# uber-research/UPSNet

Hardware: NVIDIA H100
Metric: panoptic images/sec at 1024x2048 (higher is better)
Workload: dtype bf16x3

## Files before the change

include/upsnet_b200.h:

```cpp
#ifndef UPSNET_B200_H_
#define UPSNET_B200_H_

#include <stddef.h>
#include <stdint.h>

#ifdef __cplusplus
extern "C" {
#endif

#define UPSNET_E_BADARG (-1)
#define UPSNET_E_UNSUPPORTED (-2)
#define UPSNET_E_WORKSPACE (-3)

#define UPSNET_LAYOUT_NCHW 0
#define UPSNET_LAYOUT_NHWC 1
#define UPSNET_LAYOUT_FLAT_PAIR 2

#define UPSNET_DTYPE_F32 0
#define UPSNET_DTYPE_BF16 1
#define UPSNET_DTYPE_PAIR 2

#define UPSNET_EPI_RELU 1
#define UPSNET_EPI_RES_UP2 2
#define UPSNET_EPI_STEM_PAIR 8
#define UPSNET_EPI_NO_TMA 4
#define UPSNET_EPI_PAIR_GROUP(G) ((((G) / 64) & 0xfff) << 8)
#define UPSNET_EPI_SIGMOID_FROM(c) ((((c) + 1) & 0x3ff) << 20)

#define UPSNET_PREC_FP32_SIMT 0
#define UPSNET_PREC_BF16X3 1
#define UPSNET_PREC_BF16 2

int upsnet_version(int *n_sm);

int upsnet_roi_align_forward(const void *feat, int B, int C, int H, int W, int layout, int dtype,
                             const float *rois, int R, int PH, int PW, int sampling_ratio,
                             float spatial_scale, void *out, void *stream);

int upsnet_roi_align_fpn_forward(const void *const feats[4], const int Hs[4], const int Ws[4],
                                 const float scales[4], int B, int C, int layout, int dtype,
                                 const float *rois, int R, int PH, int PW, int sampling_ratio,
                                 void *out, int *levels_out, const int *n_dev, void *stream);

int upsnet_nms_workspace_bytes(int S, int max_seg_len, size_t *bytes);
int upsnet_nms_segmented(const float *boxes, const int *seg_offsets, int S, int max_seg_len,
                         float thresh, int *keep_out, int *keep_cnt, void *workspace,
                         size_t workspace_bytes, void *stream);
int upsnet_nms_host(int *keep_out, int *num_out, const float *boxes_host, int boxes_num,
                    int boxes_dim, float thresh, int device_id);

int upsnet_dcn_forward(const float *x, const float *offset, const float *mask,
                       const float *weight, const float *bias, float *y, int N, int Cin, int H,
                       int W, int Cout, int kh, int kw, int stride_h, int stride_w, int pad_h,
                       int pad_w, int dil_h, int dil_w, int deformable_groups, int epi_flags,
                       int precision, void *stream);

int upsnet_conv2d_forward(const float *x, const float *weight, const float *bias,
                          const float *residual, float *y, int N, int Cin, int H, int W,
                          int Cout, int kh, int kw, int stride_h, int stride_w, int pad_h,
                          int pad_w, int dil_h, int dil_w, int epi_flags, int precision,
                          void *stream);

int upsnet_igemm_packed_weight_bytes(int Cout, int Cin, int kh, int kw, size_t *bytes);
int upsnet_igemm_pack_weight(const float *weight, int Cout, int Cin, int kh, int kw, void *packed,
                             void *stream);
int upsnet_igemm_forward(const void *x_nhwc, const float *offset, const float *mask,
                         const void *packed, const float *bias, const void *residual, void *y,
                         int N, int H, int W, int Cin, int Cout, int kh, int kw, int stride_h,
                         int stride_w, int pad_h, int pad_w, int dil_h, int dil_w, int out_layout,
                         int x_dtype, int y_dtype, int epi_flags, int precision, const int *n_dev, void *stream);
int upsnet_tma_set_tile_n(int bn);

int upsnet_dcn_packed_weight_bytes(int Cout, int Cin, int kh, int kw, size_t *bytes);
int upsnet_dcn_pack_weight(const float *weight, int Cout, int Cin, int kh, int kw, void *packed, void *stream);
int upsnet_dcn_pair_forward(const void *x_pair, const float *offset, const float *mask, const void *packed,
                            const float *bias, void *y_pair, int N, int H, int W, int Cin, int Cout, int kh, int kw,
                            int pad_h, int pad_w, int dil_h, int dil_w, int epi_flags, void *stream);
int upsnet_dcn_set_tile_n(int bn);

int upsnet_panoptic_workspace_bytes(int n, int H, int W, int num_thing, size_t *bytes);
int upsnet_panoptic_workspace_min_bytes(int n, int H, int W, int num_thing, size_t *bytes);
int upsnet_panoptic_head(const float *fcn, int S, int H, int W, const float *boxes,
                         const float *cls_prob, const float *mask_logit, const int64_t *cls_idx,
                         int n, const int *n_dev, int num_stuff, double fraction_threshold, int64_t *keep_out,
                         int *k_out, int64_t *labels, int64_t *sem_labels, void *workspace,
                         size_t workspace_bytes, void *stream);
int upsnet_panoptic_head_up4(const float *score, int S, int Hs, int Ws, const float *boxes,
                             const float *cls_prob, const float *mask_logit, const int64_t *cls_idx,
                             int n, const int *n_dev, int num_stuff, double fraction_threshold, int64_t *keep_out,
                             int *k_out, int64_t *labels, int64_t *sem_labels, void *workspace,
                             size_t workspace_bytes, void *stream);

int upsnet_mask_removal(const float *boxes, const float *cls_prob, const float *mask_logit,
                        const int64_t *cls_idx, int n, const int *n_dev, int H, int W, int num_thing,
                        double fraction_threshold, int64_t *keep_out, int *k_out, float *mask_energy,
                        void *workspace, size_t workspace_bytes, void *stream);

int upsnet_stem_workspace_bytes(int N, int H, int W, int kh, int kw, int pad, size_t *bytes);
int upsnet_stem_packed_weight_bytes(int Cout, int kh, size_t *bytes);
int upsnet_stem_pack_weight(const float *weight, int Cout, int Cin, int kh, int kw, void *packed,
                            void *stream);
int upsnet_stem_forward(const float *x, const void *packed_w, const float *bias, void *y, int N, int Cin,
                        int H, int W, int Cout, int kh, int kw, int pad, int epi_flags, void *workspace,
                        size_t workspace_bytes, void *stream);

int upsnet_maxpool2d_nhwc(const void *x, void *y, int N, int H, int W, int C, int k, int stride,
                          int pad, int dtype, void *stream);

int upsnet_upsample_bilinear_nchw(const float *x, float *y, int planes, int H, int W, int factor,
                                  void *stream);

int upsnet_fcn_score_fuse(const float *s2, const float *s3, const float *s4, const float *s5, float *out,
                          int planes, int H, int W, void *stream);

int upsnet_fcn_score_fuse_backward(const float *dscore, float *ds3, float *ds4, float *ds5, int planes, int H,
                                   int W, void *stream);

int upsnet_rpn_decode(const float *const *deltas, const long long *const *top_idx, const int *k,
                      const int *hs, const int *ws, const int *strides, const double *base_anchors,
                      int L, int A, const float *im_info, float *boxes_out, void *stream);

int upsnet_rpn_topk_workspace_bytes(int L, size_t *bytes);
int upsnet_rpn_topk(const float *const *probs, const int *hs, const int *ws, int L, int A,
                    int pre_nms_top_n, float *out_scores, long long *out_idx, void *workspace,
                    size_t workspace_bytes, void *stream);

int upsnet_rpn_collect(const int *keep, const int *keep_cnt, const int *seg_offsets, const float *boxes,
                       const float *scores, int S, int max_seg_len, int post_nms_top_n, float *rois,
                       float *out_scores, unsigned char *valid, void *stream);

int upsnet_maskroi_prepare(const float *rois, const unsigned char *roi_valid, const float *bbox_delta,
                           const float *cls_prob, int R, int C, int class_agnostic, float score_thresh,
                           const float weights[4], const float *im_info, float *sc_out, int *cls_out,
                           float *bx_out, int *offs_out, void *stream);

int upsnet_maskroi_finish(const int *keep, const int *keep_cnt, const int *seg_offsets, const float *sc,
                          const int *cls, const float *bx, int nseg, int max_seg_len, int top_n, int cap,
                          float *out_sc, float *out_bx, long long *out_cls, int *n_out, void *stream);

int upsnet_mask_rows(const float *b1, const int *n1, int cap1, const float *b2, const int *n2, int cap2, float *rows,
                     int *u, int *pan_row, void *stream);

int upsnet_unified_pan_workspace_bytes(int num_seg_classes, size_t *bytes);
int upsnet_unified_pan_result(const long long *seg, const long long *pan, const long long *cls_inds, int k,
                              const int *k_dev, int H, int W, int num_seg_classes, int num_classes,
                              int stuff_area_limit, unsigned char *pan_2ch, int *err_out, void *workspace,
                              size_t workspace_bytes, void *stream);

int upsnet_prep_image(const unsigned char *image_hwc, int h, int w, double scale, int out_h, int out_w, int pad_h,
                      int pad_w, const double pixel_means[3], float *blob, int flip, void *stream);

int upsnet_label_restore(const long long *src0, const long long *src1, int Hp, int Wp, int h, int w, double fx,
                         int out_h, int out_w, long long *dst0, long long *dst1, void *stream);

#define UPSNET_PQ_MAX_GT 4096
#define UPSNET_PQ_MAX_PAIRS 65536
#define UPSNET_PQ_MAX_PRED 2048
#define UPSNET_PQ_E_PRED_CATEGORY 1
#define UPSNET_PQ_E_GT_COUNT 2
#define UPSNET_PQ_E_PAIRS 4
#define UPSNET_PQ_E_GT_TABLE 8
#define UPSNET_PQ_E_PRED_COUNT 16
#define UPSNET_PQ_E_MATCHES 32
int upsnet_pq_workspace_bytes(size_t *bytes);
int upsnet_pq_update(const unsigned char *pan_2ch, const unsigned char *gt_rgb, int H, int W, const long long *gt_table,
                     int num_gt, const unsigned char *cat_flags, long long *acc_counts, double *acc_iou, int *err,
                     void *workspace, size_t workspace_bytes, void *stream);

#define UPSNET_SSEG_MAX_CLASSES 224
int upsnet_sseg_update(const void *pred, int pred_bytes, int pred_pitch, const int *row_src, const int *col_src,
                       const unsigned char *gt, int H, int W, int num_classes, long long *acc, void *stream);

#define UPSNET_COCOEVAL_MAX_DET 2048
#define UPSNET_COCOEVAL_MAX_GT 1024
#define UPSNET_COCOEVAL_MAX_GT_CAT 192
#define UPSNET_COCOEVAL_MAX_CATEGORIES 256
#define UPSNET_COCOEVAL_MAX_IMAGES (1 << 17)
#define UPSNET_COCOEVAL_E_DET_COUNT 1
#define UPSNET_COCOEVAL_E_GT_COUNT 2
#define UPSNET_COCOEVAL_E_GT_CAT 4
#define UPSNET_COCOEVAL_E_CLASS 8
#define UPSNET_COCOEVAL_E_RECORDS 16
#define UPSNET_COCOEVAL_E_RLE_SIZE 32
typedef struct {
  float score;
  int category;
  int image;
  int rank;
  unsigned long long matched, ignored;
} upsnet_coco_record;
int upsnet_cocoeval_workspace_bytes(int n, int cap, long long gt_counts_total, size_t *bytes);
int upsnet_cocoeval_image(int segm, const float *boxes, const float *scores, const int64_t *cls_inds, int n,
                          const int *n_dev, const uint32_t *counts, int cap, const int *run_len, int H, int W,
                          const double *gt_table, int num_gt, const uint32_t *gt_counts, const int64_t *gt_offsets,
                          int num_categories, const int *class_to_k, int image_slot, upsnet_coco_record *records,
                          int record_cap, int *n_records, long long *npig, int *err, void *workspace,
                          size_t workspace_bytes, void *stream);
#define UPSNET_GT_RLE_E_CAPACITY 64
int upsnet_gt_rle_workspace_bytes(int num_anns, int h, int w, size_t *bytes);
int upsnet_gt_rle(int h, int w, int num_anns, const int *ann_poly, const int *poly_vert, const double *verts,
                  const int64_t *src_offsets, const uint32_t *src_counts, uint32_t *gt_counts, long long capacity,
                  int64_t *gt_offsets, int *err, void *workspace, size_t workspace_bytes, void *stream);
int upsnet_cocoeval_accumulate_workspace_bytes(int n_records, size_t *bytes);
int upsnet_cocoeval_accumulate(const upsnet_coco_record *records, int n_records, const int *image_rank,
                               const long long *npig, int num_categories, double *precision, double *recall,
                               double *scores, void *workspace, size_t workspace_bytes, void *stream);

#define UPSNET_COMBINED_MAX_DET 2048
#define UPSNET_COMBINED_E_RUN_LEN 1
#define UPSNET_COMBINED_E_RLE_SIZE 2
#define UPSNET_COMBINED_E_DET_COUNT 4
int upsnet_combined_pan_workspace_bytes(int n, int H, int W, size_t *bytes);
int upsnet_combined_pan_result(const void *sem, int sem_elem_size, int H, int W, const float *scores,
                               const int64_t *cls_inds, int n, const int *n_dev, const uint32_t *counts, int cap,
                               const int *run_len, int num_seg_classes, int num_classes, float score_threshold,
                               float fraction_threshold, int stuff_area_limit, unsigned char *pan_2ch, int *err,
                               void *workspace, size_t workspace_bytes, void *stream);

int upsnet_im_post_workspace_bytes(int n, int cap, size_t *bytes);
int upsnet_im_post_rle(const float *mask_probs, int C, int M, const float *boxes, const int64_t *cls_inds, int n,
                       const int *n_dev, int H, int W, uint32_t *counts, int cap, int *run_len, int *overflow,
                       void *workspace, size_t workspace_bytes, void *stream);

int upsnet_dcn_im2col(const float *x, const float *offset, const float *mask, int Cin, int H, int W, int kh, int kw,
                      int stride_h, int stride_w, int pad_h, int pad_w, int dil_h, int dil_w, float *col, void *stream);
int upsnet_dcn_col2im(const float *dcol, const float *offset, const float *mask, int Cin, int H, int W, int kh, int kw,
                      int stride_h, int stride_w, int pad_h, int pad_w, int dil_h, int dil_w, float *dx, void *stream);
int upsnet_dcn_col2im_coord(const float *dcol, const float *x, const float *offset, const float *mask, int Cin, int H,
                            int W, int kh, int kw, int stride_h, int stride_w, int pad_h, int pad_w, int dil_h, int dil_w,
                            float *doffset, float *dmask, void *stream);

int upsnet_roi_align_backward(const float *dout, const float *rois, int R, int B, int C, int H, int W, int PH, int PW,
                              int sampling_ratio, float spatial_scale, float *dfeat, void *stream);

#define UPSNET_RPN_TARGETS_MAX_G 4096
int upsnet_rpn_targets_workspace_bytes(long long num_anchors, int batch_size, size_t *bytes);
int upsnet_rpn_targets(const float *gt_boxes, int G, const double *cell_anchors, const int *strides,
                       const int *field_sizes, int L, int A, double im_height, double im_width, double straddle_thresh,
                       float positive_overlap, float negative_overlap, int batch_size, int num_fg, unsigned long long seed,
                       int64_t *labels, float *bbox_targets, float *inside_weights, float *outside_weights, int *counts,
                       void *workspace, size_t workspace_bytes, void *stream);

int upsnet_proposal_targets_workspace_bytes(int num_rois, int num_gt, int batch_rois, size_t *bytes);
int upsnet_proposal_targets(const float *rois, int R, const float *gt_boxes, const float *gt_max_overlaps,
                            const int *gt_max_classes, const int *gt_classes, const int *gt_box_to_gt_ind, int G,
                            const float *obj_boxes, const int *obj_poly_off, const int *poly_vert_off, const float *verts,
                            int num_objects, float im_scale, int num_classes, int batch_rois, int fg_per_image,
                            float fg_thresh, float bg_thresh_hi, float bg_thresh_lo, float wx, float wy, float ww,
                            float wh, int cls_agnostic_bbox_reg, int mask_size, unsigned long long seed, float *rois_out,
                            int64_t *labels, float *bbox_targets, float *bbox_inside_weights,
                            float *bbox_outside_weights, int64_t *nongt_inds, float *mask_rois, float *mask_int32,
                            unsigned char *roi_has_mask, int *counts, void *workspace, size_t workspace_bytes,
                            void *stream);

int upsnet_panoptic_loss_workspace_bytes(int k, int h, int w, size_t *bytes);
int upsnet_panoptic_loss_forward(const float *fcn_score, int S, int h, int w, const float *mask_score, int k, int C,
                                 int mask_size, const float *gt_rois, const int64_t *cls_idx, const int64_t *seg_gt,
                                 const void *mask_gt, int mask_gt_is_int64, int G, const int64_t *keep_inds,
                                 int num_classes, int enable_void, float box_scale, float *loss, float *accuracy,
                                 int *counts, float *lse, int *gt_channel, void *workspace, size_t workspace_bytes,
                                 void *stream);
int upsnet_panoptic_loss_backward(const float *fcn_score, int S, int h, int w, const float *mask_score, int k, int C,
                                  int mask_size, const float *gt_rois, const int64_t *cls_idx, int num_classes,
                                  int enable_void, float box_scale, const float *lse, const int *gt_channel,
                                  const float *grad_out, float *d_fcn_score, float *d_mask_score, void *workspace,
                                  size_t workspace_bytes, void *stream);

int upsnet_panoptic_gt(const int64_t *seg_gt, const void *mask_gt, int mask_gt_is_int64, int G, const int64_t *keep_inds,
                       int k, int h, int w, int num_seg_classes, int num_classes, int64_t *panoptic_gt, void *stream);

int upsnet_draw_keys(unsigned long long seed, int stream_id, int n, unsigned long long *keys, void *stream);

int upsnet_semantic_loss_workspace_bytes(int h, int w, size_t *bytes);
int upsnet_semantic_loss_forward(const float *fcn_score, int S, int h, int w, const void *seg_gt, int seg_gt_is_int64,
                                 float *loss, int *counts, float *lse, void *workspace, size_t workspace_bytes,
                                 void *stream);
int upsnet_semantic_loss_backward(const float *fcn_score, int S, int h, int w, const void *seg_gt, int seg_gt_is_int64,
                                  const float *lse, const int *counts, const float *grad_out, float *d_fcn_score,
                                  void *stream);

int upsnet_fcn_roi_loss_workspace_bytes(int S, int R, int M, int backward, size_t *bytes);
int upsnet_fcn_roi_loss_forward(const float *fcn_score, const float *bias, int S, int h, int w, const float *rois, int R,
                                const void *seg_roi_gt, int seg_roi_gt_is_int64, int M, int sampling_ratio,
                                float spatial_scale, float *loss, int *counts, float *lse, void *workspace,
                                size_t workspace_bytes, void *stream);
int upsnet_fcn_roi_loss_backward(const float *fcn_score, const float *bias, int S, int h, int w, const float *rois, int R,
                                 const void *seg_roi_gt, int seg_roi_gt_is_int64, int M, int sampling_ratio,
                                 float spatial_scale, const float *lse, const float *grad_out, float *d_fcn_score,
                                 float *d_bias, void *workspace, size_t workspace_bytes, void *stream);

int upsnet_rpn_loss_workspace_bytes(int num_anchors, size_t *bytes);
int upsnet_rpn_loss_forward(int num_levels, int A, const int *h, const int *w, const float *const *cls_score,
                            const float *const *bbox_pred, const int64_t *const *labels, const long long *label_strides,
                            const float *const *bbox_targets, const float *const *bbox_inside_weights,
                            const float *const *bbox_outside_weights, const long long *bbox_strides,
                            float rpn_batch_size, float *cls_loss, float *bbox_loss, void *workspace,
                            size_t workspace_bytes, void *stream);
int upsnet_rpn_loss_backward(int num_levels, int A, const int *h, const int *w, const float *const *cls_score,
                             const float *const *bbox_pred, const int64_t *const *labels, const long long *label_strides,
                             const float *const *bbox_targets, const float *const *bbox_inside_weights,
                             const float *const *bbox_outside_weights, const long long *bbox_strides,
                             float rpn_batch_size, const float *grad_cls, const float *grad_bbox,
                             float *const *d_cls_score, float *const *d_bbox_pred, void *stream);

int upsnet_mask_rcnn_loss_workspace_bytes(int R, int B, long long mask_numel, size_t *bytes);
int upsnet_mask_rcnn_loss_forward(const float *cls_score, const int64_t *cls_label, int R, int K, const float *bbox_pred,
                                  const float *bbox_target, const float *bbox_inside_weight,
                                  const float *bbox_outside_weight, int B, const float *mask_score,
                                  const float *mask_target, long long mask_numel, float *cls_loss, float *bbox_loss,
                                  float *mask_loss, float *accuracy, int *counts, void *workspace,
                                  size_t workspace_bytes, void *stream);
int upsnet_mask_rcnn_loss_backward(const float *cls_score, const int64_t *cls_label, int R, int K, const float *bbox_pred,
                                   const float *bbox_target, const float *bbox_inside_weight,
                                   const float *bbox_outside_weight, int B, const float *mask_score,
                                   const float *mask_target, long long mask_numel, const int *counts,
                                   const float *grad_cls, const float *grad_bbox, const float *grad_mask,
                                   float *d_cls_score, float *d_bbox_pred, float *d_mask_score, void *stream);

#define UPSNET_LABELS_MAX_POLY_VERTS 1024
#define UPSNET_LABELS_MAX_OBJ_VERTS 1536
#define UPSNET_LABELS_MAX_G 65535
int upsnet_training_labels(const unsigned char* label, int h0, int w0, const int* seg_rows, int Hs, const int* seg_cols,
                           int Ws, int64_t* seg_gt, const int* q_rows, int Hq, const int* q_cols, int Wq,
                           int64_t* seg_gt_4x, const int* m_rows, int Hm, const int* m_cols, int Wm, const int* obj_poly,
                           const int* poly_vert, const int* verts, const int* obj_yrange, int G, int max_poly_verts,
                           int max_obj_verts, void* mask_gt, int mask_gt_is_int64, const int* roi_rows,
                           const int* roi_cols, int n_roi, int M, int64_t* seg_roi_gt, void* stream);

#define UPSNET_SGD_MAX_GROUPS 16
#define UPSNET_SGD_CHUNK 8192
#define UPSNET_SGD_GRAD_F32 0
#define UPSNET_SGD_GRAD_BF16 1
#define UPSNET_SGD_GRAD_NONE 2
typedef struct {
  float *param;
  float *buf;
  const void *grad;
  int n;
  int group;
  int kind;
  float inv_world;
} upsnet_sgd_chunk;
typedef struct {
  const float *grad;
  void *out;
  int n;
  int reserved;
} upsnet_sgd_pack_chunk;
int upsnet_sgd_apply(const upsnet_sgd_chunk *chunks, int num_chunks, int num_groups, const double *group_lr,
                     const float *group_weight_decay, const float *group_momentum, double lr, const double *lr_table,
                     const unsigned char *decay_table, const int *iteration, int table_begin, int table_len,
                     void *stream);
int upsnet_sgd_pack(const upsnet_sgd_pack_chunk *chunks, int num_chunks, void *stream);
int upsnet_sgd_advance(int *iteration, void *stream);

#define UPSNET_GRAD_RELU 1
#define UPSNET_GRAD_RES_UP2 2
#define UPSNET_GRAD_UNSHUFFLE2 4
#define UPSNET_GRAD_DY_NHWC 8
int upsnet_conv_grad_prepare_workspace_bytes(int N, int C, int H, int W, int flags, size_t *bytes);
int upsnet_conv_grad_prepare(const float *dy, const float *y, void *g, float *dbias, float *dres, int N, int C, int H,
                             int W, int flags, int precision, void *workspace, size_t workspace_bytes, void *stream);
int upsnet_igemm_packed_weight_dgrad_bytes(int Cout, int Cin, int kh, int kw, size_t *bytes);
int upsnet_igemm_pack_weight_dgrad(const float *weight, int Cout, int Cin, int kh, int kw, void *packed, void *stream);
int upsnet_conv_dgrad_scatter2(const float *dxc, float *dx, int N, int H, int W, int C, void *stream);
int upsnet_conv_wgrad_workspace_bytes(int N, int H, int W, int Cin, int Cout, int kh, int kw, int stride_h, int stride_w,
                                      int pad_h, int pad_w, int dil_h, int dil_w, int precision, size_t *bytes);
int upsnet_conv_wgrad(const void *x_nhwc, const void *g, float *dw, int N, int H, int W, int Cin, int Cout, int kh, int kw,
                      int stride_h, int stride_w, int pad_h, int pad_w, int dil_h, int dil_w, int flags, int precision,
                      void *workspace, size_t workspace_bytes, void *stream);

int upsnet_group_norm_workspace_bytes(int N, int C, int H, int W, int groups, size_t *bytes);
int upsnet_group_norm_forward(const void *x, const float *gamma, const float *beta, const float *shift,
// ... 14 lines not shown
```

upsnet_b200/csrc/capi.cu:

```cuda
#include "common.cuh"
#include "tc_params.cuh"

namespace ups {
struct ConvParams {
  const float* x; const float* offset; const float* mask; const float* weight;
  const float* bias; const float* residual; float* y;
  int N, Cin, H, W, Cout, kh, kw, sh, sw, ph, pw, dh, dw, dg, Ho, Wo, relu;
};
int launch_igemm_simt(const ConvParams& p, cudaStream_t stream);

}

extern "C" int upsnet_version(int* n_sm) {
  if (n_sm) {
    int dev = 0, sms = 0;
    if (cudaGetDevice(&dev) == cudaSuccess &&
        cudaDeviceGetAttribute(&sms, cudaDevAttrMultiProcessorCount, dev) == cudaSuccess)
      *n_sm = sms;
    else
      *n_sm = -1;
  }
  return 90;
}

static int conv_common(const float* x, const float* offset, const float* mask, const float* weight,
                       const float* bias, const float* residual, float* y, int N, int Cin, int H,
                       int W, int Cout, int kh, int kw, int sh, int sw, int ph, int pw, int dh,
                       int dw, int dg, int epi_flags, int precision, void* stream) {
  if (!x || !weight || !y) return UPSNET_E_BADARG;
  if (N <= 0 || Cin <= 0 || H <= 0 || W <= 0 || Cout <= 0 || kh <= 0 || kw <= 0 || sh <= 0 ||
      sw <= 0 || ph < 0 || pw < 0 || dh <= 0 || dw <= 0 || dg <= 0 || Cin % dg != 0)
    return UPSNET_E_BADARG;
  ups::ConvParams p;
  p.x = x; p.offset = offset; p.mask = mask; p.weight = weight; p.bias = bias;
  p.residual = residual; p.y = y;
  p.N = N; p.Cin = Cin; p.H = H; p.W = W; p.Cout = Cout; p.kh = kh; p.kw = kw; p.sh = sh;
  p.sw = sw; p.ph = ph; p.pw = pw; p.dh = dh; p.dw = dw; p.dg = dg;
  p.Ho = ups::conv_out_size(H, ph, dh, kh, sh);
  p.Wo = ups::conv_out_size(W, pw, dw, kw, sw);
  p.relu = (epi_flags & UPSNET_EPI_RELU) ? 1 : 0;
  if (p.Ho <= 0 || p.Wo <= 0) return UPSNET_E_BADARG;
  if ((size_t)Cin * H * W >= (1ull << 31)) return UPSNET_E_UNSUPPORTED;
  switch (precision) {
    case UPSNET_PREC_FP32_SIMT:
      return ups::launch_igemm_simt(p, (cudaStream_t)stream);
    default:
      return UPSNET_E_UNSUPPORTED;
  }
}

extern "C" int upsnet_dcn_forward(const float* x, const float* offset, const float* mask,
                                  const float* weight, const float* bias, float* y, int N, int Cin,
                                  int H, int W, int Cout, int kh, int kw, int stride_h,
                                  int stride_w, int pad_h, int pad_w, int dil_h, int dil_w,
                                  int deformable_groups, int epi_flags, int precision,
                                  void* stream) {
  if (!offset) return UPSNET_E_BADARG;
  return conv_common(x, offset, mask, weight, bias, nullptr, y, N, Cin, H, W, Cout, kh, kw,
                     stride_h, stride_w, pad_h, pad_w, dil_h, dil_w, deformable_groups, epi_flags,
                     precision, stream);
}

extern "C" int upsnet_conv2d_forward(const float* x, const float* weight, const float* bias,
                                     const float* residual, float* y, int N, int Cin, int H, int W,
                                     int Cout, int kh, int kw, int stride_h, int stride_w,
                                     int pad_h, int pad_w, int dil_h, int dil_w, int epi_flags,
                                     int precision, void* stream) {
  return conv_common(x, nullptr, nullptr, weight, bias, residual, y, N, Cin, H, W, Cout, kh, kw,
                     stride_h, stride_w, pad_h, pad_w, dil_h, dil_w, 1, epi_flags, precision,
                     stream);
}

extern "C" int upsnet_igemm_packed_weight_bytes(int Cout, int Cin, int kh, int kw, size_t* bytes) {
  if (!bytes || Cout <= 0 || Cin <= 0 || kh <= 0 || kw <= 0) return UPSNET_E_BADARG;
  if (!ups::tc_supported(Cin, kh, kw, 1)) return UPSNET_E_UNSUPPORTED;
  *bytes = ups::tc_packed_weight_bytes(Cout, Cin, kh, kw);
  return 0;
}

extern "C" int upsnet_igemm_pack_weight(const float* weight, int Cout, int Cin, int kh, int kw,
                                        void* packed, void* stream) {
  if (!weight || !packed || Cout <= 0 || Cin <= 0 || kh <= 0 || kw <= 0) return UPSNET_E_BADARG;
  if (!ups::tc_supported(Cin, kh, kw, 1)) return UPSNET_E_UNSUPPORTED;
  return ups::tc_pack_weight(weight, Cout, Cin, kh, kw, packed, (cudaStream_t)stream);
}

extern "C" int upsnet_igemm_forward(const void* x_nhwc, const float* offset, const float* mask,
                                    const void* packed, const float* bias, const void* residual,
                                    void* y, int N, int H, int W, int Cin, int Cout, int kh, int kw,
                                    int stride_h, int stride_w, int pad_h, int pad_w, int dil_h,
                                    int dil_w, int out_layout, int x_dtype, int y_dtype, int epi_flags,
                                    int precision, const int* n_dev, void* stream) {
  if (!x_nhwc || !packed || !y) return UPSNET_E_BADARG;
  if (N <= 0 || Cin <= 0 || H <= 0 || W <= 0 || Cout <= 0 || kh <= 0 || kw <= 0 || stride_h <= 0 ||
      stride_w <= 0 || pad_h < 0 || pad_w < 0 || dil_h <= 0 || dil_w <= 0)
    return UPSNET_E_BADARG;
  if (precision != UPSNET_PREC_BF16X3 && precision != UPSNET_PREC_BF16) return UPSNET_E_BADARG;
  if (out_layout != UPSNET_LAYOUT_NCHW && out_layout != UPSNET_LAYOUT_NHWC) return UPSNET_E_BADARG;
  if (mask && !offset) return UPSNET_E_BADARG;
  if ((size_t)H * W >= (1ull << 31)) return UPSNET_E_UNSUPPORTED;
  ups::TcParams p{};
  p.x = x_nhwc; p.offset = offset; p.mask = mask; p.bias = bias; p.residual = residual; p.y = y;
  p.n_dev = n_dev;
  p.N = N; p.H = H; p.W = W; p.Cin = Cin; p.Cout = Cout; p.kh = kh; p.kw = kw; p.sh = stride_h;
  p.sw = stride_w; p.ph = pad_h; p.pw = pad_w; p.dh = dil_h; p.dw = dil_w;
  p.Ho = ups::conv_out_size(H, pad_h, dil_h, kh, stride_h);
  p.Wo = ups::conv_out_size(W, pad_w, dil_w, kw, stride_w);
  if (p.Ho <= 0 || p.Wo <= 0) return UPSNET_E_BADARG;
  p.relu = (epi_flags & UPSNET_EPI_RELU) ? 1 : 0;
  p.out_nhwc = out_layout == UPSNET_LAYOUT_NHWC;
  p.res_up2 = (epi_flags & UPSNET_EPI_RES_UP2) ? 1 : 0;
  p.no_tma = (epi_flags & UPSNET_EPI_NO_TMA) ? 1 : 0;
  if (p.res_up2 && (!residual || !p.out_nhwc || (p.Ho & 1) || (p.Wo & 1))) return UPSNET_E_BADARG;
  p.x3 = precision == UPSNET_PREC_BF16X3;
  if (x_dtype < UPSNET_DTYPE_F32 || x_dtype > UPSNET_DTYPE_PAIR || y_dtype < UPSNET_DTYPE_F32 || y_dtype > UPSNET_DTYPE_PAIR)
    return UPSNET_E_BADARG;
  p.x_bf16 = x_dtype == UPSNET_DTYPE_BF16;
  p.y_bf16 = y_dtype == UPSNET_DTYPE_BF16;
  p.x_pair = x_dtype == UPSNET_DTYPE_PAIR;
  p.y_pair = y_dtype == UPSNET_DTYPE_PAIR;
  p.pair_group = 64 * ((epi_flags >> 8) & 0xfff);
  p.sig_from = ((epi_flags >> 20) & 0x3ff) - 1;
  if (p.sig_from >= 0 && (p.y_pair || p.y_bf16 || p.residual)) return UPSNET_E_UNSUPPORTED;
  if (p.x_bf16 && p.x3) return UPSNET_E_UNSUPPORTED;
  if ((p.x_pair || p.y_pair) && !p.x3) return UPSNET_E_UNSUPPORTED;
  if (p.y_pair && !p.out_nhwc) return UPSNET_E_BADARG;
  return ups::launch_igemm_tc(p, packed, (cudaStream_t)stream);
}
```

upsnet_b200/csrc/igemm_tma.cu:

```cuda
#include <cuda.h>
#include <cuda_bf16.h>
#include <cstdlib>

#include "common.cuh"
#include "tc_ptx.cuh"
#include "tc_params.cuh"

namespace ups {

constexpr int TM_EPI_WARPS = 8;
constexpr int TM_WARP_TMA = 8, TM_WARP_RES = 9;
constexpr int TM_THREADS = 10 * 32;
constexpr int TM_MAX_STAGES = 8;
constexpr int TM_SLAB_BYTES = 128 * 128;
constexpr int TM_MMA_BF16 = 0, TM_MMA_WIDE = 1;

struct TmaGeom {
  const float* bias;
  int N, Ho, Wo, Cout, Cin;
  int kw, KHW, ph, pw, dh, dw;
  int bw, bh, bn;
  int tiles_w, tiles_h, tiles_n, n_tiles;
  const int* n_dev;
  int BN, stages, relu, has_res;
  int res_up2;
  int direct, y_bf16, out_nhwc;
  void* y;
  int stem;
  int sig_from;
  int x3;
  int x_lo;
  int w_lo;
  int pg;
  int res_inplace;
  int opairs;
  int wide;
};

__device__ __forceinline__ int pair_chan(int n, int G) { return (n / G) * 2 * G + (n % G); }

struct TmaSmem {
  uint32_t stages, out, res, acc, a_bytes, b_bytes, stage_bytes, total;
  uint32_t a_half, b_half;
  uint32_t oslabs, res_slab;
};
template <int N, int W>
__device__ __forceinline__ void acc_stage_sw(const float (&d)[N / 2], float* buf, int row0) {
  const int t = threadIdx.x & 127, l = t & 31;
  const int r = row0 + 16 * (t >> 5) + (l >> 2);
#pragma unroll
  for (int i = 0; i < W / 8; ++i) {
    const int c = 8 * i + 2 * (l & 3);
#pragma unroll
    for (int h = 0; h < 2; ++h) {
      const int rr = r + 8 * h;
      const int pc = ((((c >> 2) ^ (rr & 7))) << 2) | (c & 3);
      *reinterpret_cast<float2*>(buf + (size_t)rr * W + pc) = make_float2(d[4 * i + 2 * h], d[4 * i + 2 * h + 1]);
    }
  }
}
__device__ __forceinline__ void acc_ld16_sw(uint32_t rowaddr, int row, int col, uint32_t (&r)[16]) {
#pragma unroll
  for (int i = 0; i < 4; ++i) {
    const uint32_t a = rowaddr + ((uint32_t)(((col >> 2) + i) ^ (row & 7)) << 4);
    asm volatile("ld.shared.v4.b32 {%0, %1, %2, %3}, [%4];"
                 : "=r"(r[4 * i]), "=r"(r[4 * i + 1]), "=r"(r[4 * i + 2]), "=r"(r[4 * i + 3]) : "r"(a));
  }
}
__host__ __device__ inline TmaSmem tma_smem_layout(int BN, int stages, bool has_res, bool direct, bool x3, bool res_up2,
                                                  bool res_inplace, int opairs) {
  TmaSmem s;
  const uint32_t mul = x3 ? 2u : 1u;
  s.a_half = 128 * 128; s.b_half = (uint32_t)BN * 128;
  s.a_bytes = s.a_half * mul;
  s.b_bytes = s.b_half * mul;
  s.stage_bytes = s.a_bytes + s.b_bytes;
  s.stages = 1024;
  s.out = s.stages + s.stage_bytes * (uint32_t)stages;
  s.res_slab = (x3 && res_up2) ? 4096u : (uint32_t)TM_SLAB_BYTES;
  if (x3) {
    s.oslabs = direct ? 0u : (res_inplace ? 2u * (uint32_t)(BN / 64) : (uint32_t)opairs);
    s.res = s.out + s.oslabs * 2u * TM_SLAB_BYTES;
    s.acc = s.res + ((has_res && !res_inplace) ? 2u * (uint32_t)(BN / 64) * 2u * s.res_slab : 0u);
  } else {
    s.oslabs = 0;
    const uint32_t out_slabs = direct ? 0 : (BN == 64 ? 1 : 2);
    s.res = s.out + out_slabs * TM_SLAB_BYTES;
    s.acc = s.res + (has_res ? 2u * (uint32_t)(BN / 64) * TM_SLAB_BYTES : 0u);
  }
  s.total = s.acc + ((x3 && !direct) ? 0u : 128u * (uint32_t)BN * 4u);
  return s;
}

template <int N, int MMA>
__global__ void __launch_bounds__(TM_THREADS, 1)
igemm_tma_kernel(const __grid_constant__ CUtensorMap tm_x, const __grid_constant__ CUtensorMap tm_w,
                 const __grid_constant__ CUtensorMap tm_y, const __grid_constant__ CUtensorMap tm_r, const TmaGeom g) {
  extern __shared__ __align__(1024) uint8_t smem_dyn[];
  const uint32_t raw = smem_u32(smem_dyn);
  const uint32_t base = (raw + 1023u) & ~1023u;
  uint8_t* sm = smem_dyn + (base - raw);
  const TmaSmem L = tma_smem_layout(g.BN, g.stages, g.has_res != 0, g.direct != 0, g.x3 != 0, g.res_up2 != 0, g.res_inplace != 0,
                                    g.opairs);
  const uint32_t bar_full = base, bar_empty = base + 8 * TM_MAX_STAGES;
  const uint32_t bar_rfull = bar_empty + 8 * TM_MAX_STAGES, bar_rempty = bar_rfull + 16;

  const int tid = threadIdx.x, warp = tid >> 5, lane = tid & 31;
  const int cchunks = g.Cin / 64;
  const int num_kb = g.KHW * cchunks;
  const int tiles_n = g.n_dev ? (min(max(*g.n_dev, 0), g.N) + g.bn - 1) / g.bn : g.tiles_n;
  const long long m_tiles = (long long)g.tiles_w * g.tiles_h * tiles_n;
  const long long num_tiles = m_tiles * g.n_tiles;
  const uint32_t box_bytes = (uint32_t)(g.bw * g.bh * g.bn) * 128u;

  if (tid == 0) {
    for (int s = 0; s < g.stages; ++s) {
      mbar_init(bar_full + 8 * s, 1);
      mbar_init(bar_empty + 8 * s, TM_EPI_WARPS);
    }
    for (int b = 0; b < 2; ++b) {
      mbar_init(bar_rfull + 8 * b, 1);
      mbar_init(bar_rempty + 8 * b, g.res_inplace ? 1 : TM_EPI_WARPS);
    }
    fence_mbar_init();
  } else if (warp == TM_WARP_TMA && lane == 0) {
    prefetch_tmap(&tm_x);
    prefetch_tmap(&tm_w);
    prefetch_tmap(&tm_y);
    if (g.has_res || (g.stem && g.x3)) prefetch_tmap(&tm_r);
  }
  __syncthreads();

  if (warp == TM_WARP_TMA) {
    if (lane == 0) {
      uint32_t s = 0, ph = 0;
      uint32_t a_dst = base + L.stages;
      const uint32_t tx_bytes = (g.x3 ? 2u * box_bytes : box_bytes) + L.b_bytes;
      for (long long tile = blockIdx.x; tile < num_tiles; tile += gridDim.x) {
        const int nt = (int)(tile % g.n_tiles);
        const long long mt = tile / g.n_tiles;
        const int w0 = (int)(mt % g.tiles_w) * g.bw;
        const int h0 = (int)((mt / g.tiles_w) % g.tiles_h) * g.bh;
        const int i0 = (int)(mt / ((long long)g.tiles_w * g.tiles_h)) * g.bn;
        const int n0 = nt * g.BN;
        int kbr = 0, cc = 0, kj = 0;
        int cw = w0 - g.pw, ch = h0 - g.ph;
        for (int kb = 0; kb < num_kb; ++kb) {
          const uint32_t bf = bar_full + 8 * s;
          mbar_wait(bar_empty + 8 * s, ph ^ 1u);
          mbar_arrive_expect_tx(bf, tx_bytes);
          if (g.stem)
            tma_load_5d(a_dst, &tm_x, bf, 0, w0, kbr & 1, h0 + (kbr >> 1), i0);
          else
            tma_load_4d(a_dst, &tm_x, bf, cc * 64, cw, ch, i0);
          tma_load_2d(a_dst + L.a_bytes, &tm_w, bf, kbr * 64, n0);
          if (g.x3) {
            if (g.stem)
              tma_load_5d(a_dst + L.a_half, &tm_r, bf, 0, w0, kbr & 1, h0 + (kbr >> 1), i0);
            else
              tma_load_4d(a_dst + L.a_half, &tm_x, bf, g.x_lo + cc * 64, cw, ch, i0);
            tma_load_2d(a_dst + L.a_bytes + L.b_half, &tm_w, bf, kbr * 64, g.w_lo + n0);
          }
          ++kbr;
          if (++cc == cchunks) {
            cc = 0; cw += g.dw;
            if (++kj == g.kw) { kj = 0; cw = w0 - g.pw; ch += g.dh; }
          }
          a_dst += L.stage_bytes;
          if (++s == (uint32_t)g.stages) { s = 0; ph ^= 1u; a_dst = base + L.stages; }
        }
      }
    }
    __syncwarp();
  } else if (warp == TM_WARP_RES) {
    if (lane == 0 && g.has_res) {
      uint32_t ti_local = 0;
      const int slabs = g.BN / 64;
      for (long long tile = blockIdx.x; tile < num_tiles; tile += gridDim.x, ++ti_local) {
        const int nt = (int)(tile % g.n_tiles);
        const long long mt = tile / g.n_tiles;
        const int w0 = (int)(mt % g.tiles_w) * g.bw;
        const int h0 = (int)((mt / g.tiles_w) % g.tiles_h) * g.bh;
        const int i0 = (int)(mt / ((long long)g.tiles_w * g.tiles_h)) * g.bn;
        const uint32_t rb = ti_local & 1u, ruse = ti_local >> 1;
        const uint32_t rdst = base + L.res + rb * (uint32_t)slabs * TM_SLAB_BYTES;
        mbar_wait(bar_rempty + 8 * rb, (ruse & 1u) ^ 1u);
        if (g.x3) {
          const uint32_t lo_off = g.res_inplace ? (uint32_t)TM_SLAB_BYTES : L.res_slab;
          const uint32_t pdst = g.res_inplace ? base + L.out + rb * (uint32_t)slabs * 2u * TM_SLAB_BYTES
                                              : base + L.res + rb * (uint32_t)slabs * 2u * L.res_slab;
          mbar_arrive_expect_tx(bar_rfull + 8 * rb, (g.res_up2 ? box_bytes / 4 : box_bytes) * (uint32_t)slabs * 2u);
          for (int s = 0; s < slabs; ++s) {
            const int c = pair_chan(nt * g.BN + s * 64, g.pg);
            tma_load_4d(pdst + (uint32_t)s * 2u * lo_off, &tm_r, bar_rfull + 8 * rb, c, w0 >> g.res_up2, h0 >> g.res_up2, i0);
            tma_load_4d(pdst + (uint32_t)s * 2u * lo_off + lo_off, &tm_r, bar_rfull + 8 * rb, c + g.pg, w0 >> g.res_up2,
                        h0 >> g.res_up2, i0);
          }
          continue;
        }
        mbar_arrive_expect_tx(bar_rfull + 8 * rb, (g.res_up2 ? box_bytes / 4 : box_bytes) * (uint32_t)slabs);
        for (int s = 0; s < slabs; ++s)
          tma_load_4d(rdst + s * TM_SLAB_BYTES, &tm_r, bar_rfull + 8 * rb, nt * g.BN + s * 64, w0 >> g.res_up2,
                      h0 >> g.res_up2, i0);
      }
    }
    __syncwarp();
  } else {
    const int wg = warp >> 2;
    const uint32_t dhi = wg_desc_hi(1024);
    const uint32_t a_row0 = (uint32_t)wg * 64u * 128u;
    const uint32_t ah16 = L.a_half >> 4;
    float* accbuf = reinterpret_cast<float*>(sm + L.acc);
    constexpr int SW = MMA == TM_MMA_WIDE ? N / 2 : N;
    const bool staged = MMA != TM_MMA_WIDE || g.direct;
    float d[N / 2];
    uint32_t s = 0, ph = 0;
    auto mainloop = [&]() {
      int prev = -1;
      for (int kb = 0; kb < num_kb; ++kb) {
        mbar_wait(bar_full + 8 * s, ph);
        const uint32_t st0 = base + L.stages + s * L.stage_bytes;
        const uint32_t a = wg_desc_lo(st0 + a_row0), b = wg_desc_lo(st0 + L.a_bytes);
        wgmma_fence();
#pragma unroll
        for (uint32_t k = 0; k < 4; ++k) {
          const uint32_t acc = (kb | k) ? 1u : 0u;
          if constexpr (MMA == TM_MMA_WIDE) {
            Wgmma<N>::mma(d, wg_desc(a + 2 * k, dhi), wg_desc(b + 2 * k, dhi), acc);
            Wgmma<N / 2>::mma(*reinterpret_cast<float(*)[N / 4]>(&d[0]), wg_desc(a + ah16 + 2 * k, dhi), wg_desc(b + 2 * k, dhi), 1u);
          } else {
            Wgmma<N>::mma(d, wg_desc(a + 2 * k, dhi), wg_desc(b + 2 * k, dhi), acc);
          }
        }
        wgmma_commit();
        wgmma_wait<1>();
        wgmma_fence_acc(d);
        if (prev >= 0 && lane == 0) mbar_arrive(bar_empty + 8 * prev);
        prev = (int)s;
        if (++s == (uint32_t)g.stages) { s = 0; ph ^= 1u; }
      }
      wgmma_wait<0>();
      wgmma_fence_acc(d);
      if (prev >= 0 && lane == 0) mbar_arrive(bar_empty + 8 * prev);
      if constexpr (MMA == TM_MMA_WIDE) {
#pragma unroll
        for (int i = 0; i < N / 4; ++i) { d[i] += d[N / 4 + i]; d[N / 4 + i] = 0.f; }
      }
      if (staged) {
        named_bar(3, 256);
        acc_stage_sw<N, SW>(d, accbuf, wg * 64);
        named_bar(3, 256);
      }
    };
    const int q = warp & 3, half = warp >> 2;
    const int row = q * 32 + lane;
    const uint32_t trow = smem_u32(accbuf + (size_t)row * SW);
    const int units = g.BN / 32;
    const int upw = units >= 4 ? units / 2 : 1;
    const int bar_id = g.BN == 64 ? 1 : 1 + half;
    const int bar_cnt = g.BN == 64 ? 256 : 128;
    const bool leader = (g.BN == 64 ? warp == 0 : q == 0) && lane == 0;
    const uint32_t out_slab = base + L.out + (g.BN == 64 ? 0u : (uint32_t)half * TM_SLAB_BYTES);
    const uint32_t sw_row = (uint32_t)row * 128u;
    const uint32_t rx = (uint32_t)(row & 7);
    auto res_row = [&](int r) {
      if (!g.res_up2) return r;
      const int w = r % g.bw, h = (r / g.bw) % g.bh, n = r / (g.bw * g.bh);
      return (w >> 1) + (g.bw >> 1) * ((h >> 1) + (g.bh >> 1) * n);
    };
    const int rrow = res_row(row);
    const uint32_t rs_row = (uint32_t)rrow * 128u, rrx = (uint32_t)(rrow & 7);
    uint32_t fr_row[2], fr_res[2], fr_rx[2];
#pragma unroll
    for (int h = 0; h < 2; ++h) {
      const int r = wg * 64 + 16 * (warp & 3) + (lane >> 2) + 8 * h, rr = res_row(r);
      fr_row[h] = (uint32_t)r * 128u; fr_res[h] = (uint32_t)rr * 128u; fr_rx[h] = (uint32_t)(rr & 7);
    }
    uint32_t ti_local = 0, oc = 0;
    for (long long tile = blockIdx.x; tile < num_tiles; tile += gridDim.x, ++ti_local) {
      const int nt = (int)(tile % g.n_tiles);
      const long long mt = tile / g.n_tiles;
      const int w0 = (int)(mt % g.tiles_w) * g.bw;
      const int h0 = (int)((mt / g.tiles_w) % g.tiles_h) * g.bh;
      const int i0 = (int)(mt / ((long long)g.tiles_w * g.tiles_h)) * g.bn;
      const int n0 = nt * g.BN;
      const uint32_t buf = ti_local & 1u, use = ti_local >> 1;
      mainloop();
      if (g.has_res) mbar_wait(bar_rfull + 8 * buf, use & 1u);
      if (g.direct) {
        const int wq = row % g.bw, hq = (row / g.bw) % g.bh, nq = row / (g.bw * g.bh);
        const int wo = w0 + wq, ho = h0 + hq, ni = i0 + nq;
        const bool ok = nq < g.bn && wo < g.Wo && ho < g.Ho && ni < g.N;
        const size_t HoWo = (size_t)g.Ho * g.Wo;
        const size_t pix = ((size_t)ni * g.Ho + ho) * g.Wo + wo;
        const int cbeg = half * (g.BN / 2), cend = cbeg + g.BN / 2;
        for (int cb = cbeg; cb < cend; cb += 16) {
          uint32_t v[16];
          acc_ld16_sw(trow, row, cb, v);
          const int co0 = n0 + cb;
          if (!ok || co0 >= g.Cout) continue;
#pragma unroll
          for (int e = 0; e < 16; ++e) {
            const int co = co0 + e;
            if (co >= g.Cout) break;
            float o = __uint_as_float(v[e]);
            if (g.bias) o += __ldg(g.bias + co);
            if (g.relu) o = fmaxf(o, 0.f);
            if (g.sig_from >= 0 && co >= g.sig_from) o = 1.f / (1.f + expf(-o));
            const size_t oi = g.out_nhwc ? pix * g.Cout + co : ((size_t)ni * g.Cout + co) * HoWo + (size_t)ho * g.Wo + wo;
            if (g.y_bf16) reinterpret_cast<__nv_bfloat16*>(g.y)[oi] = __float2bfloat16_rn(o);
            else reinterpret_cast<float*>(g.y)[oi] = o;
          }
        }
        continue;
      }
      if constexpr (MMA == TM_MMA_WIDE) {
        const bool lead = warp == 0 && lane == 0;
        const uint32_t cq4 = (uint32_t)(lane & 3) * 4u;
        const uint32_t fx = (uint32_t)(lane >> 2);
#pragma unroll
        for (int sl = 0; sl < SW / 64; ++sl, ++oc) {
          uint32_t ob;
          if (g.res_inplace) {
            ob = base + L.out + (buf * (uint32_t)(SW / 64) + (uint32_t)sl) * 2u * TM_SLAB_BYTES;
          } else {
            ob = base + L.out + (g.opairs == 2 ? (oc & 1u) : 0u) * 2u * TM_SLAB_BYTES;
            if (lead) {
              if (g.opairs == 2) bulk_wait_read1(); else bulk_wait_read0();
            }
            named_bar(1, 256);
          }
#pragma unroll
          for (int j = 0; j < 8; ++j) {
            const int i = 8 * sl + j;
            float2 bv = make_float2(0.f, 0.f);
            if (g.bias) bv = __ldg(reinterpret_cast<const float2*>(g.bias + n0 + 8 * i) + (lane & 3));
#pragma unroll
            for (int h = 0; h < 2; ++h) {
              float a = d[4 * i + 2 * h], b = d[4 * i + 2 * h + 1];
              const uint32_t oa = ob + fr_row[h] + (((uint32_t)j ^ fx) << 4) + cq4;
              if (g.bias) { a += bv.x; b += bv.y; }
              if (g.has_res) {
                uint32_t hw, lw;
                if (g.res_inplace) { hw = lds32(oa); lw = lds32(oa + TM_SLAB_BYTES); }
                else {
                  const uint32_t ra = base + L.res + (buf * (uint32_t)(SW / 64) + (uint32_t)sl) * 2u * L.res_slab + fr_res[h];
                  hw = lds32(ra + (((uint32_t)j ^ fr_rx[h]) << 4) + cq4);
                  lw = lds32(ra + L.res_slab + (((uint32_t)j ^ fr_rx[h]) << 4) + cq4);
                }
                a += pair_x(hw, lw);
                b += pair_y(hw, lw);
              }
              if (g.relu) { a = fmaxf(a, 0.f); b = fmaxf(b, 0.f); }
              uint32_t hw, lw;
              split_pair2(a, b, hw, lw);
              sts32(oa, hw);
              sts32(oa + TM_SLAB_BYTES, lw);
            }
          }
          fence_proxy_async();
          named_bar(1, 256);
          if (lead) {
            const int c = pair_chan(n0 + sl * 64, g.pg);
            tma_store_4d(&tm_y, ob, c, w0, h0, i0);
            tma_store_4d(&tm_y, ob + TM_SLAB_BYTES, c + g.pg, w0, h0, i0);
            bulk_commit();
          }
        }
        __syncwarp();
        if (lane == 0 && g.has_res && !g.res_inplace) mbar_arrive(bar_rempty + 8 * buf);
        if (g.res_inplace && lead) {
          bulk_wait_read0();
          mbar_arrive(bar_rempty + 8 * buf);
        }
      } else {
        for (int ui = 0; ui < upw; ++ui) {
          const int u = half * upw + ui;
          const int slab = u >> 1;
          const uint32_t jb = (uint32_t)(u & 1) * 4u;
          uint32_t v0[16], v1[16];
          acc_ld16_sw(trow, row, u * 32, v0);
          acc_ld16_sw(trow, row, u * 32 + 16, v1);
          if ((u & 1) == 0 || g.BN == 64) {
            if (leader) bulk_wait_read0();
            named_bar(bar_id, bar_cnt);
          }
          float o[32];
  #pragma unroll
          for (int e = 0; e < 16; ++e) { o[e] = __uint_as_float(v0[e]); o[16 + e] = __uint_as_float(v1[e]); }
          if (g.bias) {
            const float4* bp = reinterpret_cast<const float4*>(g.bias + n0 + u * 32);
  #pragma unroll
            for (int e = 0; e < 8; ++e) {
              const float4 b4 = __ldg(bp + e);
              o[4 * e] += b4.x; o[4 * e + 1] += b4.y; o[4 * e + 2] += b4.z; o[4 * e + 3] += b4.w;
            }
          }
          if (g.has_res) {
            const uint32_t rs = base + L.res + (buf * (uint32_t)(g.BN / 64) + (uint32_t)slab) * TM_SLAB_BYTES + rs_row;
  #pragma unroll
            for (int c = 0; c < 4; ++c) {
              const uint4 rv = lds128(rs + (((jb + c) ^ rrx) << 4));
              const uint32_t rw[4] = {rv.x, rv.y, rv.z, rv.w};
  #pragma unroll
              for (int e = 0; e < 4; ++e) {
                o[c * 8 + 2 * e] += bf16x2_x(rw[e]);
                o[c * 8 + 2 * e + 1] += bf16x2_y(rw[e]);
              }
            }
          }
          if (g.relu) {
  #pragma unroll
            for (int e = 0; e < 32; ++e) o[e] = fmaxf(o[e], 0.f);
          }
  #pragma unroll
          for (int c = 0; c < 4; ++c) sts128(out_slab + sw_row + (((jb + c) ^ rx) << 4), pack_bf16x8(o + c * 8));
          if ((u & 1) == 1 || g.BN == 64) {
            fence_proxy_async();
            named_bar(bar_id, bar_cnt);
            if (leader) {
              tma_store_4d(&tm_y, out_slab, n0 + slab * 64, w0, h0, i0);
              bulk_commit();
            }
          }
        }
        __syncwarp();
        if (lane == 0 && g.has_res) mbar_arrive(bar_rempty + 8 * buf);
      }
    }
    if (leader || (g.x3 && warp == 0 && lane == 0)) bulk_wait0();
  }
}

static bool encode_bf16(EncodeTiledFn enc, CUtensorMap* tm, const void* ptr, int rank, const cuuint64_t* dims,
                        const cuuint32_t* box, const cuuint64_t* byte_strides = nullptr) {
  cuuint64_t strides[5];
  cuuint64_t acc = 2;
  for (int i = 0; i + 1 < rank; ++i) { acc *= dims[i]; strides[i] = byte_strides ? byte_strides[i] : acc; }
  const cuuint32_t es[5] = {1, 1, 1, 1, 1};
  return enc(tm, CU_TENSOR_MAP_DATA_TYPE_BFLOAT16, (cuuint32_t)rank, const_cast<void*>(ptr), dims, strides, box, es,
             CU_TENSOR_MAP_INTERLEAVE_NONE, CU_TENSOR_MAP_SWIZZLE_128B, CU_TENSOR_MAP_L2_PROMOTION_L2_256B,
             CU_TENSOR_MAP_FLOAT_OOB_FILL_NONE) == CUDA_SUCCESS;
}

static void tma_pick_box(int N, int Ho, int Wo, int kh, int kw, int dh, int dw, bool even, int* bw_o, int* bh_o, int* bn_o) {
  long long best_tiles = -1, best_halo = 0;
  int bbw = 1, bbh = 1, bbn = 1;
  const int wmax = Wo < 128 ? Wo : 128;
  for (int bw = 1; bw <= wmax; ++bw) {
    if (Wo > 32 && (bw & (bw - 1))) continue;
    if (even && (bw & 1)) continue;
    const int hmax = (128 / bw) < Ho ? (128 / bw) : Ho;
    for (int bh = 1; bh <= hmax; ++bh) {
      if (even && (bh & 1)) continue;
      int bn = 128 / (bw * bh);
      if (bn > N) bn = N;
      if (bn < 1) continue;
      const long long tiles = (long long)((Wo + bw - 1) / bw) * ((Ho + bh - 1) / bh) * ((N + bn - 1) / bn);
      const long long halo = (long long)(bw + (kw - 1) * dw) * (bh + (kh - 1) * dh) * bn;
      if (best_tiles < 0 || tiles < best_tiles || (tiles == best_tiles && (halo < best_halo || (halo == best_halo && bw > bbw)))) {
        best_tiles = tiles; best_halo = halo; bbw = bw; bbh = bh; bbn = bn;
      }
    }
  }
  *bw_o = bbw; *bh_o = bbh; *bn_o = bbn;
}

template <int N, int MMA>
static int tma_launch_n(dim3 grid, size_t smem, cudaStream_t stream, const CUtensorMap& tm_x, const CUtensorMap& tm_w,
                        const CUtensorMap& tm_y, const CUtensorMap& tm_r, const TmaGeom& g) {
  static ups::PerDeviceOnce configured;
  if (configured.need())
    UPS_CUDA(cudaFuncSetAttribute(igemm_tma_kernel<N, MMA>, cudaFuncAttributeMaxDynamicSharedMemorySize, 227 * 1024));
  igemm_tma_kernel<N, MMA><<<grid, TM_THREADS, smem, stream>>>(tm_x, tm_w, tm_y, tm_r, g);
  UPS_CHECK_LAUNCH();
  return 0;
}
static int tma_launch(int BN, dim3 grid, size_t smem, cudaStream_t stream, const CUtensorMap& tm_x, const CUtensorMap& tm_w,
                      const CUtensorMap& tm_y, const CUtensorMap& tm_r, const TmaGeom& g) {
  if (g.wide) {
    if (BN == 32) return tma_launch_n<64, TM_MMA_WIDE>(grid, smem, stream, tm_x, tm_w, tm_y, tm_r, g);
    if (BN == 64) return tma_launch_n<128, TM_MMA_WIDE>(grid, smem, stream, tm_x, tm_w, tm_y, tm_r, g);
    if (BN == 128) return tma_launch_n<256, TM_MMA_WIDE>(grid, smem, stream, tm_x, tm_w, tm_y, tm_r, g);
  } else {
    if (BN == 32) return tma_launch_n<32, TM_MMA_BF16>(grid, smem, stream, tm_x, tm_w, tm_y, tm_r, g);
    if (BN == 64) return tma_launch_n<64, TM_MMA_BF16>(grid, smem, stream, tm_x, tm_w, tm_y, tm_r, g);
    if (BN == 128) return tma_launch_n<128, TM_MMA_BF16>(grid, smem, stream, tm_x, tm_w, tm_y, tm_r, g);
  }
  return UPSNET_E_UNSUPPORTED;
}

static bool tma_fit(int BN, bool has_res, bool direct, bool pair, bool res_up2, bool res_inplace, int* stages, int* opairs,
                    TmaSmem* L) {
  const uint32_t cap = 227 * 1024 - 1024;
  auto lay = [&](int st, int op) { return tma_smem_layout(BN, st, has_res, direct, pair, res_up2, res_inplace, op); };
  int st = TM_MAX_STAGES, op = 2;
  while (st > 2 && lay(st, op).total > cap) --st;
  if (pair && !direct && !res_inplace && (st < 4 || lay(st, op).total > cap)) {
    int st1 = 4;
    while (st1 > 2 && lay(st1, 1).total > cap) --st1;
    if (st1 > st || lay(st, op).total > cap) { st = st1; op = 1; }
  }
  *stages = st; *opairs = op; *L = lay(st, op);
  return L->total <= cap;
}

static int g_tma_force_bn = 0;

int launch_igemm_tma(const TcParams& p, const void* packed, cudaStream_t stream) {
  if (p.no_tma || p.offset) return UPSNET_E_UNSUPPORTED;
  const bool pair = p.x_pair != 0;
  if (pair != (p.x3 != 0) || (!pair && !p.x_bf16)) return UPSNET_E_UNSUPPORTED;
  if (p.y_pair && (!pair || !p.out_nhwc || (p.Cout % 64) != 0)) return UPSNET_E_UNSUPPORTED;
  if (pair && p.y_bf16) return UPSNET_E_UNSUPPORTED;
  const int pg = p.y_pair ? (p.pair_group > 0 ? p.pair_group : p.Cout) : 0;
  if (p.y_pair && ((pg % 64) != 0 || (p.Cout % pg) != 0)) return UPSNET_E_UNSUPPORTED;
  const bool direct = (!p.y_bf16 && !p.y_pair) || !p.out_nhwc || (p.Cout % 64) != 0;
  if (p.sig_from >= 0 && !direct) return UPSNET_E_UNSUPPORTED;
  if (direct && (p.residual || p.Cout > 256)) return UPSNET_E_UNSUPPORTED;
  if (p.res_up2 && (!p.residual || (p.Ho & 1) || (p.Wo & 1))) return UPSNET_E_UNSUPPORTED;
  const bool strided = p.sh != 1 || p.sw != 1;
  if (strided && (p.kh != 1 || p.kw != 1 || p.ph != 0 || p.pw != 0)) return UPSNET_E_UNSUPPORTED;
  if ((p.Cin % 64) || (!direct && (p.Cout % 64)) || p.kh * p.kw > 49) return UPSNET_E_UNSUPPORTED;
  if ((((uintptr_t)p.x) & 15) || (((uintptr_t)p.y) & 15) || (((uintptr_t)packed) & 15) || (p.residual && (((uintptr_t)p.residual) & 15)))
    return UPSNET_E_UNSUPPORTED;
  if (p.bias && (((uintptr_t)p.bias) & 15)) return UPSNET_E_UNSUPPORTED;
  EncodeTiledFn enc = tma_encoder();
  if (!enc) return UPSNET_E_UNSUPPORTED;
  const int sms = num_sms();
  TmaGeom g{};
  g.bias = p.bias;
  g.N = p.N; g.Ho = p.Ho; g.Wo = p.Wo; g.Cout = p.Cout; g.Cin = p.Cin;
  g.kw = p.kw; g.KHW = p.kh * p.kw; g.ph = p.ph; g.pw = p.pw; g.dh = p.dh; g.dw = p.dw;
  g.relu = p.relu; g.has_res = p.residual ? 1 : 0; g.res_up2 = p.res_up2 ? 1 : 0; g.sig_from = p.sig_from;
  g.n_dev = p.n_dev;
  tma_pick_box(p.N, p.Ho, p.Wo, p.kh, p.kw, p.dh, p.dw, g.res_up2 != 0, &g.bw, &g.bh, &g.bn);
  g.tiles_w = (p.Wo + g.bw - 1) / g.bw;
  g.tiles_h = (p.Ho + g.bh - 1) / g.bh;
  g.tiles_n = (p.N + g.bn - 1) / g.bn;
  const long long m_tiles = (long long)g.tiles_w * g.tiles_h * g.tiles_n;
  const int Cout_pad = cout_pad(p.Cout);
  int BN = (Cout_pad % 128 == 0) ? 128 : (Cout_pad % 64 == 0 ? 64 : 32);
  g.x3 = pair ? 1 : 0; g.x_lo = p.Cin; g.w_lo = Cout_pad; g.pg = pg;
  g.res_inplace = (pair && g.has_res && !g.res_up2) ? 1 : 0;
  g.opairs = 2;
  if (g_tma_force_bn && Cout_pad % g_tma_force_bn == 0) {
    BN = g_tma_force_bn;
  } else {
    while (BN > 64 && m_tiles * (Cout_pad / BN) < 88) BN /= 2;
  }
  g.direct = direct ? 1 : 0; g.y_bf16 = p.y_bf16; g.out_nhwc = p.out_nhwc; g.y = p.y;
  TmaSmem L;
  bool ok = tma_fit(BN, g.has_res != 0, direct, pair, g.res_up2 != 0, g.res_inplace != 0, &g.stages, &g.opairs, &L);
  while (BN > 64 && (!ok || (pair && g.stages < 3))) {
    BN /= 2;
    ok = tma_fit(BN, g.has_res != 0, direct, pair, g.res_up2 != 0, g.res_inplace != 0, &g.stages, &g.opairs, &L);
  }
  if (!ok) return UPSNET_E_UNSUPPORTED;
  g.BN = BN;
  g.n_tiles = Cout_pad / BN;

  const int Kp = g.KHW * p.Cin;
  CUtensorMap tm_x, tm_w, tm_y, tm_r;
  {
    const cuuint64_t xm = pair ? 2 : 1;
    const cuuint64_t dx[4] = {(cuuint64_t)p.Cin * xm, (cuuint64_t)(strided ? p.Wo : p.W), (cuuint64_t)(strided ? p.Ho : p.H),
                              (cuuint64_t)p.N};
    const cuuint64_t sx[3] = {(cuuint64_t)p.sw * p.Cin * 2 * xm, (cuuint64_t)p.sh * p.W * p.Cin * 2 * xm,
                              (cuuint64_t)p.H * p.W * p.Cin * 2 * xm};
    const cuuint64_t dy[4] = {(cuuint64_t)p.Cout * xm, (cuuint64_t)p.Wo, (cuuint64_t)p.Ho, (cuuint64_t)p.N};
    const cuuint64_t dwt[2] = {(cuuint64_t)Kp, (cuuint64_t)Cout_pad * xm};
    const cuuint32_t box[4] = {64, (cuuint32_t)g.bw, (cuuint32_t)g.bh, (cuuint32_t)g.bn};
    const cuuint32_t boxw[2] = {64, (cuuint32_t)BN};
    if (!encode_bf16(enc, &tm_x, p.x, 4, dx, box, sx)) return UPSNET_E_UNSUPPORTED;
    if (!encode_bf16(enc, &tm_w, packed, 2, dwt, boxw)) return UPSNET_E_UNSUPPORTED;
    if (direct) {
      tm_y = tm_x;
      tm_r = tm_x;
    } else {
    if (!encode_bf16(enc, &tm_y, p.y, 4, dy, box)) return UPSNET_E_UNSUPPORTED;
    if (g.res_up2) {
      const cuuint64_t dr[4] = {(cuuint64_t)p.Cout * xm, (cuuint64_t)(p.Wo / 2), (cuuint64_t)(p.Ho / 2), (cuuint64_t)p.N};
      const cuuint32_t boxr[4] = {64, (cuuint32_t)(g.bw / 2), (cuuint32_t)(g.bh / 2), (cuuint32_t)g.bn};
      if (!encode_bf16(enc, &tm_r, p.residual, 4, dr, boxr)) return UPSNET_E_UNSUPPORTED;
    } else if (!encode_bf16(enc, &tm_r, p.residual ? p.residual : p.y, 4, dy, box)) {
      return UPSNET_E_UNSUPPORTED;
    }
    }
  }
  const long long num_tiles = m_tiles * g.n_tiles;
  if (num_tiles <= 0) return 0;
  g.wide = pair ? 1 : 0;
  dim3 grid((unsigned)(num_tiles < sms ? num_tiles : sms));
  return tma_launch(BN, grid, L.total + 1024, stream, tm_x, tm_w, tm_y, tm_r, g);
}


__global__ void stem_pack_image_kernel(const float* __restrict__ x, uint4* __restrict__ xp, uint4* __restrict__ xp_lo, int N, int C,
                                       int H, int W, int pad, int Hp, int Wp) {
  const long long total = (long long)N * Hp * Wp;
  for (long long t = (long long)blockIdx.x * blockDim.x + threadIdx.x; t < total; t += (long long)gridDim.x * blockDim.x) {
    const int c = (int)(t % Wp);
    const long long rest = t / Wp;
    const int r = (int)(rest % Hp), n = (int)(rest / Hp);
    const int hi = r - pad, wi = c - pad;
    float v[8] = {0.f, 0.f, 0.f, 0.f, 0.f, 0.f, 0.f, 0.f};
    if (hi >= 0 && hi < H && wi >= 0 && wi < W)
      for (int ch = 0; ch < C; ++ch) v[ch] = __ldg(x + (((size_t)n * C + ch) * H + hi) * W + wi);
    const uint4 o = pack_bf16x8(v);
    xp[t] = o;
    if (xp_lo) xp_lo[t] = pair_lo8(v, o);
  }
}

__global__ void stem_pack_weight_kernel(const float* __restrict__ w, int Cout, int Cin, int kh, int kw,
                                        __nv_bfloat16* __restrict__ packed) {
  const int total = Cout * kh * 64;
  for (int i = blockIdx.x * blockDim.x + threadIdx.x; i < total; i += gridDim.x * blockDim.x) {
    const int c = i & 7, kx = (i >> 3) & 7, ky = (i >> 6) % kh, co = i / (64 * kh);
    const float v = (c < Cin && kx < kw) ? w[(((size_t)co * Cin + c) * kh + ky) * kw + kx] : 0.f;
    __nv_bfloat16 h, l;
    split_bf16(v, h, l);
    packed[i] = h;
    packed[total + i] = l;
  }
}

static void stem_geometry(int H, int W, int kh, int kw, int pad, int* Ho, int* Wo, int* Hp, int* Wp) {
  *Ho = (H + 2 * pad - kh) / 2 + 1;
  *Wo = (W + 2 * pad - kw) / 2 + 1;
  *Hp = 2 * (*Ho + (kh >> 1));
  *Wp = 2 * *Wo + 8;
}

inline size_t stem_layout(int N, int Hp, int Wp, bool pair, void* base, uint4** hi, uint4** lo) {
  WsCarve c(base);
  const size_t pixels = (size_t)N * Hp * Wp;
  *hi = c.take<uint4>(pixels);
  *lo = pair ? c.take<uint4>(pixels) : nullptr;
  return c.bytes();
}

}

extern "C" int upsnet_tma_set_tile_n(int bn) {
  if (bn != 0 && bn != 64 && bn != 128) return UPSNET_E_BADARG;
  ups::g_tma_force_bn = bn;
  return 0;
}

extern "C" int upsnet_stem_workspace_bytes(int N, int H, int W, int kh, int kw, int pad, size_t* bytes) {
  if (!bytes || N <= 0 || H <= 0 || W <= 0 || kh <= 0 || kw <= 0 || kw > 8 || pad < 0) return UPSNET_E_BADARG;
  int Ho, Wo, Hp, Wp;
  ups::stem_geometry(H, W, kh, kw, pad, &Ho, &Wo, &Hp, &Wp);
  if (Ho <= 0 || Wo <= 0) return UPSNET_E_BADARG;
  uint4 *hi, *lo;
  *bytes = ups::stem_layout(N, Hp, Wp, true, nullptr, &hi, &lo);
  return 0;
}

extern "C" int upsnet_stem_packed_weight_bytes(int Cout, int kh, size_t* bytes) {
  if (!bytes || Cout <= 0 || kh <= 0) return UPSNET_E_BADARG;
  *bytes = (size_t)Cout * kh * 64 * 2 * 2;
  return 0;
}

extern "C" int upsnet_stem_pack_weight(const float* weight, int Cout, int Cin, int kh, int kw, void* packed, void* stream) {
  if (!weight || !packed || Cout <= 0 || Cin <= 0 || Cin > 8 || kh <= 0 || kw <= 0 || kw > 8) return UPSNET_E_BADARG;
  const int total = Cout * kh * 64;
  ups::stem_pack_weight_kernel<<<(total + 255) / 256, 256, 0, (cudaStream_t)stream>>>(weight, Cout, Cin, kh, kw,
                                                                                         (__nv_bfloat16*)packed);
  UPS_CHECK_LAUNCH();
  return 0;
}

extern "C" int upsnet_stem_forward(const float* x, const void* packed_w, const float* bias, void* y, int N, int Cin, int H,
                                   int W, int Cout, int kh, int kw, int pad, int epi_flags, void* workspace,
                                   size_t workspace_bytes, void* stream) {
  using namespace ups;
  if (!x || !packed_w || !y || !workspace) return UPSNET_E_BADARG;
  if (N <= 0 || Cin <= 0 || Cin > 8 || H <= 0 || W <= 0 || kh <= 0 || kw <= 0 || kw > 8 || pad < 0) return UPSNET_E_BADARG;
  if ((Cout % 64) || Cout > 256 || kh > 16) return UPSNET_E_UNSUPPORTED;
  if ((((uintptr_t)y) & 15) || (((uintptr_t)packed_w) & 15) || (((uintptr_t)workspace) & 15)) return UPSNET_E_BADARG;
  if (bias && (((uintptr_t)bias) & 15)) return UPSNET_E_UNSUPPORTED;
  int Ho, Wo, Hp, Wp;
  stem_geometry(H, W, kh, kw, pad, &Ho, &Wo, &Hp, &Wp);
  if (Ho <= 0 || Wo <= 0) return UPSNET_E_BADARG;
  const bool pair = (epi_flags & UPSNET_EPI_STEM_PAIR) != 0;
  uint4 *x_hi, *x_lo;
  if (workspace_bytes < stem_layout(N, Hp, Wp, pair, workspace, &x_hi, &x_lo)) return UPSNET_E_WORKSPACE;
  EncodeTiledFn enc = tma_encoder();
  if (!enc) return UPSNET_E_UNSUPPORTED;
  cudaStream_t st = (cudaStream_t)stream;
  TmaGeom g{};
  g.bias = bias;
  g.N = N; g.Ho = Ho; g.Wo = Wo; g.Cout = Cout; g.Cin = 64;
  g.kw = 1; g.KHW = kh; g.ph = 0; g.pw = 0; g.dh = 1; g.dw = 1;
  g.relu = (epi_flags & UPSNET_EPI_RELU) ? 1 : 0;
  g.sig_from = -1;
  g.stem = 1; g.y = y; g.y_bf16 = 1; g.out_nhwc = 1;
  g.x3 = pair ? 1 : 0; g.w_lo = Cout; g.pg = Cout; g.opairs = 2; g.x_lo = 0;
  tma_pick_box(N, Ho, Wo, 1, 1, 1, 1, false, &g.bw, &g.bh, &g.bn);
  g.tiles_w = (Wo + g.bw - 1) / g.bw;
  g.tiles_h = (Ho + g.bh - 1) / g.bh;
  g.tiles_n = (N + g.bn - 1) / g.bn;
  g.BN = (Cout % 128 == 0 && !pair) ? 128 : 64;
  g.n_tiles = Cout / g.BN;
  g.wide = pair ? 1 : 0;
  TmaSmem L;
  if (!tma_fit(g.BN, false, false, pair, false, false, &g.stages, &g.opairs, &L)) return UPSNET_E_UNSUPPORTED;
  CUtensorMap tm_x, tm_w, tm_y, tm_lo;
  {
    const cuuint64_t pitch = (cuuint64_t)Wp * 16;
    const cuuint64_t dx[5] = {64, (cuuint64_t)Wo, 2, (cuuint64_t)(Hp / 2), (cuuint64_t)N};
    const cuuint64_t sx[4] = {32, pitch, 2 * pitch, (cuuint64_t)Hp * pitch};
    const cuuint32_t bx[5] = {64, (cuuint32_t)g.bw, 1, (cuuint32_t)g.bh, (cuuint32_t)g.bn};
    const cuuint64_t dwt[2] = {(cuuint64_t)kh * 64, (cuuint64_t)Cout * 2};
    const cuuint32_t bw2[2] = {64, (cuuint32_t)g.BN};
    const cuuint64_t dy[4] = {(cuuint64_t)Cout * (pair ? 2 : 1), (cuuint64_t)Wo, (cuuint64_t)Ho, (cuuint64_t)N};
    const cuuint32_t by[4] = {64, (cuuint32_t)g.bw, (cuuint32_t)g.bh, (cuuint32_t)g.bn};
    if (!encode_bf16(enc, &tm_x, x_hi, 5, dx, bx, sx)) return UPSNET_E_UNSUPPORTED;
    tm_lo = tm_x;
    if (pair && !encode_bf16(enc, &tm_lo, x_lo, 5, dx, bx, sx)) return UPSNET_E_UNSUPPORTED;
    if (!encode_bf16(enc, &tm_w, packed_w, 2, dwt, bw2)) return UPSNET_E_UNSUPPORTED;
    if (!encode_bf16(enc, &tm_y, y, 4, dy, by)) return UPSNET_E_UNSUPPORTED;
  }
  {
    const long long total = (long long)N * Hp * Wp;
    long long blocks = (total + 255) / 256;
    if (blocks > kNumSMs * 32) blocks = kNumSMs * 32;
    stem_pack_image_kernel<<<(unsigned)blocks, 256, 0, st>>>(x, x_hi, x_lo, N, Cin, H, W, pad, Hp, Wp);
    UPS_CHECK_LAUNCH();
  }
  const int sms = num_sms();
  const long long num_tiles = (long long)g.tiles_w * g.tiles_h * g.tiles_n * g.n_tiles;
  dim3 grid((unsigned)(num_tiles < sms ? num_tiles : sms));
  return tma_launch(g.BN, grid, L.total + 1024, st, tm_x, tm_w, tm_y, pair ? tm_lo : tm_y, g);
}
```

upsnet_b200/csrc/tc_params.cuh:

```cuda
#pragma once
#include <cuda.h>
#include <cuda_runtime.h>
#include <cstdint>

namespace ups {

inline int cout_pad(int Cout) { return Cout <= 32 ? 32 : (Cout + 63) / 64 * 64; }

typedef CUresult (*EncodeTiledFn)(CUtensorMap*, CUtensorMapDataType, cuuint32_t, void*, const cuuint64_t*, const cuuint64_t*,
                                  const cuuint32_t*, const cuuint32_t*, CUtensorMapInterleave, CUtensorMapSwizzle,
                                  CUtensorMapL2promotion, CUtensorMapFloatOOBfill);

inline EncodeTiledFn tma_encoder() {
  static EncodeTiledFn fn = nullptr;
  static bool tried = false;
  if (!tried) {
    void* p = nullptr;
    cudaDriverEntryPointQueryResult qr = cudaDriverEntryPointSymbolNotFound;
    if (cudaGetDriverEntryPoint("cuTensorMapEncodeTiled", &p, cudaEnableDefault, &qr) == cudaSuccess &&
        qr == cudaDriverEntryPointSuccess)
      fn = reinterpret_cast<EncodeTiledFn>(p);
    else
      (void)cudaGetLastError();
    tried = true;
  }
  return fn;
}

struct TcParams {
  const void* x;
  const float* offset;
  const float* mask;
  const uint16_t* w_hi;
  const uint16_t* w_lo;
  const float* bias; const void* residual; void* y;
  int N, H, W, Cin, Cout, Cout_pad, kh, kw, sh, sw, ph, pw, dh, dw, Ho, Wo;
  int relu, out_nhwc, BN, stages, x3;
  int x_bf16, y_bf16;
  int x_pair, y_pair;
  int sig_from;
  int pair_group;
  int res_up2;
  int no_tma;
  int tile_w, tile_h;
  const int* n_dev;
};

size_t tc_packed_weight_bytes(int Cout, int Cin, int kh, int kw);
int tc_pack_weight(const float* w, int Cout, int Cin, int kh, int kw, void* packed, cudaStream_t stream);
bool tc_supported(int Cin, int kh, int kw, int dg);
int launch_igemm_tc(TcParams p, const void* packed, cudaStream_t stream);
int launch_igemm_tma(const TcParams& p, const void* packed, cudaStream_t stream);

}
```

upsnet_b200/model.py:

```python
import math

import numpy as np
import torch
import torch.nn as nn
import torch.nn.functional as F

from . import _lib, training
from . import operators as ops
from .detection import MaskROI, ProposalGenerator, StaticMaskROI, StaticProposalGenerator
from .operators import DeformConv, DeformConvWithOffset


class UPSNetConfig:

    def __init__(self, **kw):
        self.num_classes = 9
        self.num_seg_classes = 19
        self.backbone_with_dconv = 100
        self.backbone_with_dilation = False
        self.backbone_with_dpyramid = False
        self.backbone_freeze_at = 2
        self.backbone_fix_bn = True
        self.fpn_feature_dim = 256
        self.fpn_with_gap = False
# ... 24 lines not shown
        self.fpn_with_norm = "none"
        self.rpn_with_norm = "none"
        self.rcnn_with_norm = "none"
        self.fcn_with_norm = "none"
        for k, v in kw.items():
            if not hasattr(self, k):
                raise AttributeError(k)
            setattr(self, k, v)

    @classmethod
    def from_reference_config(cls, config):
        def get(sec, key, default):
            d = config.get(sec, {}) if hasattr(config, "get") else getattr(config, sec, {})
            try:
                return d[key]
            except (KeyError, TypeError):
                return getattr(d, key, default)
        return cls(num_classes=int(get("dataset", "num_classes", 9)), num_seg_classes=int(get("dataset", "num_seg_classes", 19)),
                   backbone_with_dconv=int(get("network", "backbone_with_dconv", 100)),
                   backbone_with_dilation=bool(get("network", "backbone_with_dilation", False)),
                   backbone_with_dpyramid=bool(get("network", "backbone_with_dpyramid", False)),
                   backbone_freeze_at=int(get("network", "backbone_freeze_at", 2)),
                   backbone_fix_bn=bool(get("network", "backbone_fix_bn", True)),
                   fpn_feature_dim=int(get("network", "fpn_feature_dim", 256)), fpn_with_gap=bool(get("network", "fpn_with_gap", False)),
                   fcn_num_layers=int(get("network", "fcn_num_layers", 3)), num_anchors=int(get("network", "num_anchors", 3)),
                   anchor_scales=tuple(get("network", "anchor_scales", (8,))), anchor_ratios=tuple(get("network", "anchor_ratios", (0.5, 1, 2))),
                   rpn_feat_stride=tuple(get("network", "rpn_feat_stride", (4, 8, 16, 32, 64))), mask_size=int(get("network", "mask_size", 28)),
                   bbox_reg_weights=tuple(get("network", "bbox_reg_weights", (10., 10., 5., 5.))),
                   rpn_pre_nms_top_n=int(get("test", "rpn_pre_nms_top_n", 1000)), rpn_post_nms_top_n=int(get("test", "rpn_post_nms_top_n", 1000)),
                   rpn_nms_thresh=float(get("test", "rpn_nms_thresh", 0.7)), rpn_min_size=int(get("test", "rpn_min_size", 0)),
                   nms_thresh=float(get("test", "nms_thresh", 0.5)), max_det=int(get("test", "max_det", 100)),
                   score_thresh=float(get("test", "score_thresh", 0.05)), panoptic_score_thresh=float(get("test", "panoptic_score_thresh", 0.6)),
                   panoptic_box_keep_fraction=float(get("train", "panoptic_box_keep_fraction", 0.7)),
                   train_rpn_pre_nms_top_n=int(get("train", "rpn_pre_nms_top_n", 2000)),
                   train_rpn_post_nms_top_n=int(get("train", "rpn_post_nms_top_n", 2000)),
                   train_rpn_nms_thresh=float(get("train", "rpn_nms_thresh", 0.7)),
                   train_rpn_min_size=int(get("train", "rpn_min_size", 0)),
                   batch_rois=int(get("train", "batch_rois", 512)), rpn_batch_size=int(get("train", "rpn_batch_size", 256)),
                   fg_fraction=float(get("train", "fg_fraction", 0.25)),
                   fcn_with_roi_loss=bool(get("train", "fcn_with_roi_loss", False)),
                   **{k: str(get("network", k, "none")) for k in NORM_KEYS})

    @classmethod
    def cityscapes_r50(cls):
        return cls()

    @classmethod
    def coco_r50(cls):
        return cls(num_classes=81, num_seg_classes=133, fpn_with_gap=True, fcn_num_layers=3, fcn_with_roi_loss=True)

    @classmethod
    def coco_r101_dcn(cls):
        return cls(num_classes=81, num_seg_classes=133, backbone_with_dconv=3, fpn_with_gap=True,
                   fcn_num_layers=3, fcn_with_roi_loss=True)


NORM_KEYS = ("fpn_with_norm", "rpn_with_norm", "rcnn_with_norm", "fcn_with_norm")


def _check_norms(cfg):
    for k in NORM_KEYS:
        v = getattr(cfg, k)
        if v not in ("none", "group_norm", "batch_norm"):
            raise _lib.UpsnetError("network.%s: %r is not one of 'none', 'group_norm', 'batch_norm'" % (k, v))
        if v == "batch_norm" and k != "rpn_with_norm":
            raise _lib.UpsnetError("network.%s = 'batch_norm' is not built: the reference's BatchNorm2d comes from its "
                                   "absent distbatchnorm module (SyncBN); use 'group_norm' or 'none'" % k)


def _gn_conv(cin, cout, k, padding=0):
    return nn.Sequential(nn.Conv2d(cin, cout, k, padding=padding, bias=False), nn.GroupNorm(32, cout))


def _fold_bn(conv_w, bn):
    with torch.no_grad():
        scale = bn.weight / torch.sqrt(bn.running_var + bn.eps)
        shift = (bn.bias - bn.running_mean * scale).contiguous()
    return (conv_w * scale.view(-1, 1, 1, 1)).contiguous(), shift


class Bottleneck(nn.Module):

    def __init__(self, inplanes, planes, stride=1, dilation=1, downsample=None, deformable=False):
        super().__init__()
        self.conv1 = nn.Conv2d(inplanes, planes, 1, stride=stride, bias=False)
        self.bn1 = nn.BatchNorm2d(planes)
        self.deformable = deformable
        if deformable:
            self.conv2_offset = nn.Conv2d(planes, 18, 3, 1, 1)
            self.conv2_offset.weight.data.zero_()
            self.conv2_offset.bias.data.zero_()
            self.conv2 = DeformConv(planes, planes, 3, stride=1, padding=dilation, dilation=dilation, bias=False)
        else:
            self.conv2 = nn.Conv2d(planes, planes, 3, 1, dilation, dilation, bias=False)
        self.bn2 = nn.BatchNorm2d(planes)
        self.conv3 = nn.Conv2d(planes, planes * 4, 1, bias=False)
        self.bn3 = nn.BatchNorm2d(planes * 4)
        self.downsample = downsample
        self.stride, self.dilation = stride, dilation
        self._f = None

    def prepare(self):
        f = {}
        f["w1"], f["b1"] = _fold_bn(self.conv1.weight, self.bn1)
        f["w2"], f["b2"] = _fold_bn(self.conv2.weight, self.bn2)
        f["w3"], f["b3"] = _fold_bn(self.conv3.weight, self.bn3)
        if self.downsample is not None:
            f["wd"], f["bd"] = _fold_bn(self.downsample[0].weight, self.downsample[1])
        self._f = {k: v.detach() for k, v in f.items()}

    def forward(self, x):
        f = self._f
        out = ops.conv2d(x, f["w1"], f["b1"], stride=self.stride, relu=True)
        if self.deformable:
            offset = ops.conv2d(out, self.conv2_offset.weight, self.conv2_offset.bias, 1, 1, 1, out_format="nchw")
            out = ops.deform_conv(out, offset, f["w2"], f["b2"], 1, self.dilation, self.dilation, relu=True)
        else:
            out = ops.conv2d(out, f["w2"], f["b2"], 1, self.dilation, self.dilation, relu=True)
        residual = x if self.downsample is None else ops.conv2d(x, f["wd"], f["bd"], stride=self.stride)
        return ops.conv2d(out, f["w3"], f["b3"], residual=residual, relu=True)

    def forward_train(self, x, prec):
        w1, b1 = _fold_bn(self.conv1.weight, self.bn1)
        out = training.conv2d(x, w1, b1, stride=self.stride, relu=True, precision=prec)
        w2, b2 = _fold_bn(self.conv2.weight, self.bn2)
        if self.deformable:
            offset = training.OffsetConvFunction.apply(out, self.conv2_offset.weight, self.conv2_offset.bias)
            out = F.relu(training.DeformConvFunction.apply(out, offset, w2, b2, 1, self.dilation, self.dilation))
        else:
            out = training.conv2d(out, w2, b2, 1, self.dilation, self.dilation, relu=True, precision=prec)
        residual = x
        if self.downsample is not None:
            wd, bd = _fold_bn(self.downsample[0].weight, self.downsample[1])
            residual = training.conv2d(x, wd, bd, stride=self.stride, precision=prec)
        w3, b3 = _fold_bn(self.conv3.weight, self.bn3)
        return training.conv2d(out, w3, b3, residual=residual, relu=True, precision=prec)


class Stem(nn.Module):

    def __init__(self):
        super().__init__()
        self.conv1 = nn.Conv2d(3, 64, 7, 2, 3, bias=False)
        self.bn1 = nn.BatchNorm2d(64)
        self._f = None

    def prepare(self):
        w, b = _fold_bn(self.conv1.weight, self.bn1)
        self._f = (w.detach(), b.detach())

    def forward(self, x):
        stream = ops._stream()
        if x.is_cuda and stream != "f32":
            x = ops.stem_conv(x, self._f[0], self._f[1], 3, relu=True, pair=stream == "pair")
        else:
            x = ops.conv2d(x, self._f[0], self._f[1], stride=2, padding=3, relu=True)
        return ops.max_pool2d(x, 3, 2, 1)


class ResBlock(nn.Module):

    def __init__(self, planes, blocks, stride=1, dilation=1, deformable=False, with_dpyramid=False):
        super().__init__()
        inplanes = planes * 2 if planes != 64 else planes
        downsample = None
        if stride != 1 or inplanes != planes * 4:
            downsample = nn.Sequential(nn.Conv2d(inplanes, planes * 4, 1, stride=stride, bias=False),
                                       nn.BatchNorm2d(planes * 4))
        layers = [Bottleneck(inplanes, planes, stride, dilation, downsample, deformable)]
        for _ in range(1, blocks - 1):
            layers.append(Bottleneck(planes * 4, planes, dilation=dilation, deformable=deformable))
        layers.append(Bottleneck(planes * 4, planes, dilation=dilation, deformable=deformable or with_dpyramid))
        self.layers = nn.Sequential(*layers)

    def forward(self, x):
        return self.layers(x)


class ResNetBackbone(nn.Module):

    def __init__(self, blocks, cfg):
        super().__init__()
        d = cfg.backbone_with_dconv
        self.conv1 = Stem()
        self.res2 = ResBlock(64, blocks[0])
        self.res3 = ResBlock(128, blocks[1], 2, deformable=d <= 3, with_dpyramid=cfg.backbone_with_dpyramid)
        self.res4 = ResBlock(256, blocks[2], 2, deformable=d <= 4, with_dpyramid=cfg.backbone_with_dpyramid)
        s5, d5 = (1, 2) if cfg.backbone_with_dilation else (2, 1)
        self.res5 = ResBlock(512, blocks[3], s5, d5, deformable=d <= 5)

    def forward(self, x):
        c1 = self.conv1(x)
        r2 = self.res2(c1)
        r3 = self.res3(r2)
        r4 = self.res4(r3)
        return r2, r3, r4, self.res5(r4)

    def forward_train(self, x, prec):
        with torch.no_grad():
            for m in [self.conv1] + list(self.res2.layers):
                m.prepare()
            r = ops.as_float(self.res2(self.conv1(x))).float()
        out = [r]
        for stage in (self.res3, self.res4, self.res5):
            for blk in stage.layers:
                r = blk.forward_train(r, prec)
            out.append(r)
        return tuple(out)


class FPN(nn.Module):

    def __init__(self, feature_dim, with_gap, with_norm="none"):
        super().__init__()
        self.feature_dim = feature_dim
        self.gn = with_norm == "group_norm"
        if with_gap:
            self.fpn_gap = nn.Linear(2048, feature_dim)
        for name, cin in (("fpn_p5_1x1", 2048), ("fpn_p4_1x1", 1024), ("fpn_p3_1x1", 512), ("fpn_p2_1x1", 256)):
            setattr(self, name, _gn_conv(cin, feature_dim, 1) if self.gn else nn.Conv2d(cin, feature_dim, 1))
        for name in ("fpn_p5", "fpn_p4", "fpn_p3", "fpn_p2"):
            setattr(self, name, _gn_conv(feature_dim, feature_dim, 3, 1) if self.gn else
                    nn.Conv2d(feature_dim, feature_dim, 3, padding=1))
        for m in self.modules():
            if isinstance(m, nn.Conv2d):
                nn.init.kaiming_uniform_(m.weight.data, a=1)
                if m.bias is not None:
                    m.bias.data.zero_()

    def forward(self, res2, res3, res4, res5):
        def step(name, x, padding=0, residual=None, shift=None):
            up = {"residual": residual, "residual_up2": residual is not None}
            if not self.gn:
                m = getattr(self, name)
                return ops.conv2d(x, m.weight, m.bias, padding=padding, **up)
            conv, gn = getattr(self, name)
            t = ops.conv2d(x, conv.weight, None, padding=padding)
            return ops.group_norm(t, gn.weight, gn.bias, gn.num_groups, gn.eps, shift=shift, **up)

        def gap():
            return ops.linear(res5.float().mean(dim=(2, 3)), self.fpn_gap.weight, self.fpn_gap.bias, out_dtype=torch.float32)
        with_gap = hasattr(self, "fpn_gap")
        p5_1x1 = step("fpn_p5_1x1", res5, shift=gap() if with_gap and self.gn else None)
        if with_gap and not self.gn:
            g = gap().view(-1, self.feature_dim, 1, 1)
            if isinstance(p5_1x1, ops.Pair):
                p5_1x1 = ops.Pair.from_float(p5_1x1.float() + g)
            else:
                p5_1x1 = p5_1x1 + g.to(p5_1x1.dtype)
        p4_plus = step("fpn_p4_1x1", res4, residual=p5_1x1)
        p3_plus = step("fpn_p3_1x1", res3, residual=p4_plus)
        p2_plus = step("fpn_p2_1x1", res2, residual=p3_plus)
        p5 = step("fpn_p5", p5_1x1, padding=1)
        p4 = step("fpn_p4", p4_plus, padding=1)
        p3 = step("fpn_p3", p3_plus, padding=1)
        p2 = step("fpn_p2", p2_plus, padding=1)
        p6 = ops.subsample2(p5)
        return p2, p3, p4, p5, p6

    def forward_train(self, res2, res3, res4, res5, prec):
        def step(name, x, padding=0, residual=None, shift=None):
            if not self.gn:
                m = getattr(self, name)
                bias = m.bias if shift is None else m.bias + shift.reshape(self.feature_dim)
                return training.conv2d(x, m.weight, bias, padding=padding, residual=residual,
                                       residual_up2=residual is not None, precision=prec)
            conv, gn = getattr(self, name)
            t = training.conv2d(x, conv.weight, None, padding=padding, precision=prec)
            return training.group_norm(t, gn.weight, gn.bias, gn.num_groups, gn.eps, residual=residual, shift=shift)

        gap = None
        if hasattr(self, "fpn_gap"):
            gap = training.linear(res5.mean((2, 3)), self.fpn_gap.weight, self.fpn_gap.bias, precision=prec)
        p5_1x1 = step("fpn_p5_1x1", res5, shift=gap)
        p4_plus = step("fpn_p4_1x1", res4, residual=p5_1x1)
        p3_plus = step("fpn_p3_1x1", res3, residual=p4_plus)
        p2_plus = step("fpn_p2_1x1", res2, residual=p3_plus)
        p2 = step("fpn_p2", p2_plus, padding=1)
        p3 = step("fpn_p3", p3_plus, padding=1)
        p4 = step("fpn_p4", p4_plus, padding=1)
        p5 = step("fpn_p5", p5_1x1, padding=1)
        return p2, p3, p4, p5, p5[:, :, ::2, ::2]


class RPN(nn.Module):

    def __init__(self, num_anchors, input_dim):
        super().__init__()
        self.num_anchors = num_anchors
        self.conv_proposal = nn.Sequential(nn.Conv2d(input_dim, input_dim, 3, padding=1), nn.ReLU(inplace=True))
        self.cls_score = nn.Conv2d(input_dim, num_anchors, 1)
        self.bbox_pred = nn.Conv2d(input_dim, num_anchors * 4, 1)
        for m in (self.conv_proposal[0], self.cls_score, self.bbox_pred):
            nn.init.normal_(m.weight.data, 0, 0.01)
            m.bias.data.zero_()
        self._f = None

    def prepare(self):
        self._f = (torch.cat([self.cls_score.weight, self.bbox_pred.weight, self.cls_score.weight]).detach().contiguous(),
                   torch.cat([self.cls_score.bias, self.bbox_pred.bias, self.cls_score.bias]).detach().contiguous())

    def forward(self, x):
        c = self.conv_proposal[0]
        t = ops.conv2d(x, c.weight, c.bias, padding=1, relu=True)
        A = self.num_anchors
        both = ops.conv2d(t, self._f[0], self._f[1], out_format="nchw", sigmoid_from=5 * A).float()
        return both[:, :A], both[:, A:5 * A], both[:, 5 * A:]

    def forward_train(self, x, prec):
        c = self.conv_proposal[0]
        t = training.conv2d(x, c.weight, c.bias, padding=1, relu=True, precision=prec)
        return (training.conv2d(t, self.cls_score.weight, self.cls_score.bias, precision=prec),
                training.conv2d(t, self.bbox_pred.weight, self.bbox_pred.bias, precision=prec))


class RCNN(nn.Module):

    def __init__(self, num_classes, num_reg_classes, pool_size=7, dim_in=256, dim_hidden=1024, with_norm="none"):
        super().__init__()
        self.pool_size = pool_size
        self.roi_pooling = ops.FPNRoIAlign(pool_size, pool_size, [1.0 / 4, 1.0 / 8, 1.0 / 16, 1.0 / 32])
        self.gn = with_norm == "group_norm"
        if self.gn:
            self.fc6 = nn.Sequential(nn.Linear(pool_size ** 2 * dim_in, dim_hidden), nn.Unflatten(1, (dim_hidden, 1, 1)),
                                     nn.GroupNorm(32, dim_hidden), nn.Flatten(), nn.ReLU(inplace=True))
        else:
            self.fc6 = nn.Sequential(nn.Linear(pool_size ** 2 * dim_in, dim_hidden), nn.ReLU(inplace=True))
        self.fc7 = nn.Sequential(nn.Linear(dim_hidden, dim_hidden), nn.ReLU(inplace=True))
        self.cls_score = nn.Linear(dim_hidden, num_classes)
        self.bbox_pred = nn.Linear(dim_hidden, num_reg_classes * 4)
        for m in (self.fc6[0], self.fc7[0]):
            nn.init.kaiming_uniform_(m.weight.data, a=1)
            m.bias.data.fill_(0)
        nn.init.normal_(self.cls_score.weight.data, 0, 0.01)
        self.cls_score.bias.data.fill_(0)
        nn.init.normal_(self.bbox_pred.weight.data, 0, 0.001)
        self.bbox_pred.bias.data.fill_(0)
        self.num_classes = num_classes
        self._f = None

    def prepare(self):
        self._f = (torch.cat([self.cls_score.weight, self.bbox_pred.weight]).detach().contiguous(),
                   torch.cat([self.cls_score.bias, self.bbox_pred.bias]).detach().contiguous())
        w6 = self.fc6[0].weight.detach()
        ps = self.pool_size
        self._w6_nhwc = w6.view(w6.shape[0], -1, ps, ps).permute(0, 2, 3, 1).reshape(w6.shape[0], -1).contiguous()

    def forward(self, feat, rois):
        if isinstance(feat[0], ops.Pair):
            ps = self.pool_size
            x = ops.fpn_roi_align(list(feat), rois, ps, ps, self.roi_pooling.spatial_scale, layout="flat_pair")
            w6 = self._w6_nhwc
        else:
            pool = self.roi_pooling(feat, rois)
            nhwc = pool.permute(0, 2, 3, 1)
            if self._f is not None and nhwc.is_contiguous() and not pool.is_contiguous():
                x, w6 = nhwc.reshape(pool.size(0), -1), self._w6_nhwc
            else:
                x, w6 = pool.reshape(pool.size(0), -1), self.fc6[0].weight
        fc6 = ops.linear(x, w6, self.fc6[0].bias, relu=not self.gn)
        if self.gn:
            gn = self.fc6[2]
            fc6 = ops.group_norm_rows(fc6, gn.weight, gn.bias, gn.num_groups, gn.eps, relu=True)
        fc7 = ops.linear(fc6, self.fc7[0].weight, self.fc7[0].bias, relu=True)
        both = ops.linear(fc7, self._f[0], self._f[1], out_dtype=torch.float32).float()
        return {"cls_score": both[:, :self.num_classes].contiguous(),
                "bbox_pred": both[:, self.num_classes:].contiguous(), "fc_feat": fc7}

    def forward_train(self, feat, rois, prec):
        ps = self.pool_size
        pool = training.FPNRoIAlignFunction.apply(rois, ps, ps, self.roi_pooling.spatial_scale, 2, *feat)
        fc6 = training.linear(pool.reshape(pool.shape[0], -1), self.fc6[0].weight, self.fc6[0].bias, relu=not self.gn,
                              precision=prec)
        if self.gn:
            gn = self.fc6[2]
            fc6 = training.group_norm(fc6, gn.weight, gn.bias, gn.num_groups, gn.eps, relu=True)
        fc7 = training.linear(fc6, self.fc7[0].weight, self.fc7[0].bias, relu=True, precision=prec)
        return (training.linear(fc7, self.cls_score.weight, self.cls_score.bias, precision=prec),
                training.linear(fc7, self.bbox_pred.weight, self.bbox_pred.bias, precision=prec))


class MaskBranch(nn.Module):

    def __init__(self, num_classes, mask_size=28, dim_in=256, dim_hidden=256, with_norm="none"):
        super().__init__()
        self.roi_pooling = ops.FPNRoIAlign(mask_size // 2, mask_size // 2, [1.0 / 4, 1.0 / 8, 1.0 / 16, 1.0 / 32])
        self.gn = with_norm == "group_norm"
        for i, cin in enumerate((dim_in, dim_hidden, dim_hidden, dim_hidden), start=1):
            layers = [nn.Conv2d(cin, dim_hidden, 3, 1, 1, bias=False), nn.GroupNorm(32, dim_hidden)] if self.gn else \
                [nn.Conv2d(cin, dim_hidden, 3, 1, 1)]
            setattr(self, "mask_conv%d" % i, nn.Sequential(*layers, nn.ReLU(inplace=True)))
        self.mask_deconv1 = nn.Sequential(nn.ConvTranspose2d(dim_hidden, dim_hidden, 2, 2, 0), nn.ReLU(inplace=True))
        self.mask_score = nn.Conv2d(dim_hidden, num_classes, 1)
        for m in self.modules():
            if isinstance(m, (nn.Conv2d, nn.ConvTranspose2d)):
                nn.init.kaiming_normal_(m.weight.data, mode="fan_in")
                if m.bias is not None:
                    m.bias.data.zero_()
        self._f = None

    def prepare(self):
        w = self.mask_deconv1[0].weight
        cin, cout = w.shape[0], w.shape[1]
        w1 = w.permute(2, 3, 1, 0).reshape(4 * cout, cin, 1, 1).detach().contiguous()
        b1 = self.mask_deconv1[0].bias.repeat(4).detach().contiguous()
        self._f = (w1, b1, cout)

    def forward(self, feat, rois, n_dev=None):
        bound = {} if n_dev is None else {"n_dev": n_dev}
        if n_dev is None or not isinstance(feat[0], ops.Pair):
            x = self.roi_pooling(feat, rois)
        else:
            r = self.roi_pooling
            x = ops.fpn_roi_align(list(feat), rois, r.pooled_height, r.pooled_width, r.spatial_scale, layout="auto", **bound)
        for i in range(1, 5):
            c = getattr(self, "mask_conv%d" % i)
            x = ops.conv2d(x, c[0].weight, c[0].bias, padding=1, relu=not self.gn, **bound)
            if self.gn:
                x = ops.group_norm_rows(x, c[1].weight, c[1].bias, c[1].num_groups, c[1].eps, relu=True, n_dev=n_dev)
        w1, b1, cout = self._f
        if isinstance(x, ops.Pair):
            yv = ops.conv2d(x, w1, b1, relu=True, pair_group=cout, **bound)
            n, _, h, w4 = yv.shape
            w = w4 // 4
        else:
            y = ops.conv2d(x, w1, b1, relu=True, **bound)
            n, _, h, w = y.shape
            if not (y.is_contiguous(memory_format=torch.channels_last) and y.dim() == 4):
                y = y.reshape(n, 2, 2, cout, h, w).permute(0, 3, 4, 1, 5, 2).reshape(n, cout, 2 * h, 2 * w)
                return ops.conv2d(y, self.mask_score.weight, self.mask_score.bias, out_format="nchw", **bound)
            yv = y.permute(0, 2, 3, 1).reshape(n, h, w * 4, cout).permute(0, 3, 1, 2)
        z = ops.conv2d(yv, self.mask_score.weight, self.mask_score.bias, out_format="nhwc", out_dtype=torch.float32,
                       **bound)
        K = z.shape[1]
        z = z.permute(0, 2, 3, 1).reshape(n, h, w, 2, 2, K)
        return z.permute(0, 5, 1, 3, 2, 4).reshape(n, K, 2 * h, 2 * w)

    def forward_train(self, feat, rois, prec):
        M = self.roi_pooling.pooled_height
        if rois.shape[0] == 0:
            return feat[0].new_zeros((0, self.mask_score.weight.shape[0], 2 * M, 2 * M))
        x = training.FPNRoIAlignFunction.apply(rois, M, M, self.roi_pooling.spatial_scale, 2, *feat)
        for i in range(1, 5):
            c = getattr(self, "mask_conv%d" % i)
            x = training.conv2d(x, c[0].weight, c[0].bias, padding=1, relu=not self.gn, precision=prec)
            if self.gn:
                x = training.group_norm(x, c[1].weight, c[1].bias, c[1].num_groups, c[1].eps, relu=True)
        d = self.mask_deconv1[0]
        x = training.conv_transpose2x2(x, d.weight, d.bias, relu=True, precision=prec)
        return training.conv2d(x, self.mask_score.weight, self.mask_score.bias, precision=prec)


class FCNSubNet(nn.Module):

    def __init__(self, in_channels, out_channels, num_layers, with_norm="none"):
        super().__init__()
        assert num_layers >= 2
        self.num_layers = num_layers
        self.gn = with_norm == "group_norm"
        self.conv = nn.ModuleList()
        for i in range(num_layers):
            if i == num_layers - 2:
                layer = DeformConvWithOffset(in_channels, out_channels, 3, stride=1, padding=1, dilation=1)
                in_channels = out_channels
            else:
                layer = DeformConvWithOffset(in_channels, in_channels, 3, stride=1, padding=1, dilation=1)
            norm = [nn.GroupNorm(32, in_channels)] if self.gn else []
            self.conv.append(nn.Sequential(layer, *norm, nn.ReLU(inplace=True)))
        for m in self.modules():
            if isinstance(m, nn.Conv2d):
                m.weight.data.fill_(0)
                m.bias.data.fill_(0)
            elif isinstance(m, DeformConv):
                nn.init.kaiming_normal_(m.weight.data)
                if m.bias is not None:
                    m.bias.data.fill_(0)

    def forward(self, x):
        for i in range(self.num_layers):
            l = self.conv[i][0]
            offset = ops.conv2d(x, l.conv_offset.weight, l.conv_offset.bias, 1, 1, 1, out_format="nchw")
            x = ops.deform_conv(x, offset, l.conv.weight, l.conv.bias, l.conv.stride, l.conv.padding,
                                l.conv.dilation, l.conv.deformable_groups, relu=not self.gn)
            if self.gn:
                gn = self.conv[i][1]
                x = ops.group_norm(x, gn.weight, gn.bias, gn.num_groups, gn.eps, relu=True)
        return x

    def forward_train(self, x):
        for i in range(self.num_layers):
            x = self.conv[i][0](x)
            if self.gn:
                gn = self.conv[i][1]
                x = training.group_norm(x, gn.weight, gn.bias, gn.num_groups, gn.eps, relu=True)
            else:
                x = F.relu(x)
        return x


class FCNHead(nn.Module):

    def __init__(self, in_channels, num_classes, num_layers, upsample_rate=4, with_norm="none"):
        super().__init__()
        self.fcn_subnet = FCNSubNet(in_channels, 128, num_layers, with_norm)
        self.upsample_rate = upsample_rate
        self.score = nn.Conv2d(512, num_classes, 1)
        nn.init.normal_(self.score.weight.data, 0, 0.01)
        self.score.bias.data.zero_()
        self.overlap_levels = False
        self._streams = None
        self._f = None

    def prepare(self):
        w = self.score.weight.detach()
        self._f = [w[:, 128 * l:128 * (l + 1)].contiguous() for l in range(4)]

    def _subnets(self, p2, p3, p4, p5):
        if not (p2.is_cuda and self.overlap_levels):
            return tuple(self.fcn_subnet(p) for p in (p2, p3, p4, p5))
        cur = torch.cuda.current_stream(p2.device)
        if self._streams is None:
            self._streams = [torch.cuda.Stream(device=p2.device) for _ in range(2)]
        fork = torch.cuda.Event()
        fork.record(cur)
        outs, joins = {}, []
        for st, (name, p) in zip(self._streams, (("p4", p4), ("p5", p5))):
            st.wait_event(fork)
            with torch.cuda.stream(st):
                outs[name] = self.fcn_subnet(p)
                ev = torch.cuda.Event()
                ev.record(st)
            joins.append(ev)
            if not torch.cuda.is_current_stream_capturing():
                outs[name].record_stream(cur)
        o2 = self.fcn_subnet(p2)
        o3 = self.fcn_subnet(p3)
        for ev in joins:
            cur.wait_event(ev)
        return o2, o3, outs["p4"], outs["p5"]

    def forward(self, p2, p3, p4, p5, score_only=False):
        p2, p3, p4, p5 = self._subnets(p2, p3, p4, p5)
        if self._f is not None:
            score = ops.conv2d(p2, self._f[0], self.score.bias, out_format="nchw").float()
            parts = [ops.conv2d(feat, self._f[l], None, out_format="nchw").float() for l, feat in enumerate((p3, p4, p5), start=1)]
            if score.is_cuda and score.shape[2] % 8 == 0 and score.shape[3] % 8 == 0 and \
                    all(tuple(s_.shape[2:]) == (score.shape[2] >> l, score.shape[3] >> l) for l, s_ in enumerate(parts, start=1)):
                score = ops.fcn_score_fuse(score, *parts)
            else:
                for l, s_l in enumerate(parts, start=1):
                    score = score + F.interpolate(s_l, None, 2 ** l, mode="bilinear", align_corners=False)
            ret = {"fcn_score": score}
            if self.upsample_rate != 1 and not (score_only and self.upsample_rate == 4):
                ret["fcn_output"] = ops.upsample_bilinear(score, self.upsample_rate)
            return ret
        p3 = F.interpolate(p3, None, 2, mode="bilinear", align_corners=False)
        p4 = F.interpolate(p4, None, 4, mode="bilinear", align_corners=False)
        p5 = F.interpolate(p5, None, 8, mode="bilinear", align_corners=False)
        feat = torch.cat([p2, p3, p4, p5], dim=1)
        score = ops.conv2d(feat, self.score.weight, self.score.bias, out_format="nchw")
        ret = {"fcn_score": score, "fcn_feat": feat}
        if self.upsample_rate != 1:
            ret["fcn_output"] = F.interpolate(score, None, self.upsample_rate, mode="bilinear", align_corners=False)
        return ret

    def forward_train(self, p2, p3, p4, p5, prec):
        w = self.score.weight
        scores = []
        for l, feat in enumerate((p2, p3, p4, p5)):
            feat = self.fcn_subnet.forward_train(feat)
            scores.append(training.conv2d(feat, w[:, 128 * l:128 * (l + 1)], self.score.bias if l == 0 else None,
                                          precision=prec))
        return training.FcnScoreFuseFunction.apply(*scores)


class resnet_upsnet(nn.Module):

    def __init__(self, backbone_depth, cfg=None):
        super().__init__()
        cfg = cfg or UPSNetConfig()
        self.cfg = cfg
        self.num_classes, self.num_seg_classes = cfg.num_classes, cfg.num_seg_classes
        self.num_reg_classes = cfg.num_classes
        _check_norms(cfg)
        self.resnet_backbone = ResNetBackbone(backbone_depth, cfg)
        self.fpn = FPN(cfg.fpn_feature_dim, cfg.fpn_with_gap, cfg.fpn_with_norm)
        self.rpn = RPN(cfg.num_anchors, cfg.fpn_feature_dim)
        self.rcnn = RCNN(self.num_classes, self.num_reg_classes, dim_in=cfg.fpn_feature_dim, with_norm=cfg.rcnn_with_norm)
        self.mask_branch = MaskBranch(self.num_classes, cfg.mask_size, dim_in=cfg.fpn_feature_dim,
                                      with_norm=cfg.rcnn_with_norm)
        self.fcn_head = FCNHead(cfg.fpn_feature_dim, self.num_seg_classes, cfg.fcn_num_layers,
                                with_norm=cfg.fcn_with_norm)
        self.enable_void = cfg.panoptic_box_keep_fraction < 1
        assert self.enable_void, "all shipped configs enable the void channel"
        self.pyramid_proposal = ProposalGenerator(cfg.rpn_feat_stride, cfg.anchor_scales, cfg.anchor_ratios,
                                                  cfg.rpn_pre_nms_top_n, cfg.rpn_post_nms_top_n,
                                                  cfg.rpn_nms_thresh, cfg.rpn_min_size)
        self.pyramid_proposal_train = ProposalGenerator(cfg.rpn_feat_stride, cfg.anchor_scales, cfg.anchor_ratios,
                                                        cfg.train_rpn_pre_nms_top_n, cfg.train_rpn_post_nms_top_n,
                                                        cfg.train_rpn_nms_thresh, cfg.train_rpn_min_size)
        self.mask_roi = MaskROI(cfg.max_det, self.num_classes, cfg.nms_thresh, False, cfg.score_thresh,
                                cfg.bbox_reg_weights)
        self.mask_roi_panoptic = MaskROI(cfg.max_det, self.num_classes, 0.5, True, cfg.panoptic_score_thresh,
                                         cfg.bbox_reg_weights)
        self.panoptic_head = ops.PanopticHead(self.num_seg_classes, self.num_classes, 0.3)
        self.pyramid_proposal_static = StaticProposalGenerator(cfg.rpn_feat_stride, cfg.anchor_scales,
                                                               cfg.anchor_ratios, cfg.rpn_pre_nms_top_n,
                                                               cfg.rpn_post_nms_top_n, cfg.rpn_nms_thresh,
                                                               cfg.rpn_min_size)
        self.mask_roi_static = StaticMaskROI(cfg.max_det, self.num_classes, cfg.nms_thresh, False, cfg.score_thresh,
                                             cfg.bbox_reg_weights)
        self.mask_roi_panoptic_static = StaticMaskROI(cfg.max_det, self.num_classes, 0.5, True,
                                                      cfg.panoptic_score_thresh, cfg.bbox_reg_weights)
        self.static_engine = True
        self.use_cuda_graph = True
        self.overlap_heads = True
        self.dedup_mask_rows = True
        self._side = {}
        self._graphs = {}
        self._pools = {}
        self.max_graphs = 128
        self._prepared = False
        self.eval()
        bb = self.resnet_backbone
        frozen = [bb.conv1] + [getattr(bb, "res%d" % i) for i in range(2, cfg.backbone_freeze_at + 1)]
        if cfg.backbone_fix_bn:
            frozen += [m for m in self.modules() if isinstance(m, nn.BatchNorm2d)]
        for m in frozen:
            for p in m.parameters():
                p.requires_grad_(False)

    def prepare(self):
        ops.forget_packed(self.parameters())
        for m in self.modules():
            if m is not self and hasattr(m, "prepare"):
                m.prepare()
        self._prepared = True
        return self

    def _apply(self, fn, *a, **kw):
        r = super()._apply(fn, *a, **kw)
        self._prepared = False
        self._graphs, self._pools = {}, {}
        return r

    _COCO2CITY_THING = {0: 0, 1: 1, 2: -1, 3: 3, 4: 8, 5: 6, 6: 7, 7: 4, 8: 2}
    _COCO2CITY_SEG = {0: 20, 1: 43, 2: 49, 3: 51, 4: 37, 5: -1, 6: 62, 7: -1, 8: 36, 9: -1, 10: 39, 11: 53, 12: -1, 13: 55,
                      14: 60, 15: 58, 16: 59, 17: 56, 18: 54}

    @staticmethod
    def name_mapping(name, resume=False):
        if resume:
            return name[len("module."):] if name.startswith("module.") else name
        if name.startswith("conv1") or name.startswith("bn1"):
            return "resnet_backbone.conv1." + name
        return name.replace("layer1", "resnet_backbone.res2.layers").replace("layer2", "resnet_backbone.res3.layers") \
                   .replace("layer3", "resnet_backbone.res4.layers").replace("layer4", "resnet_backbone.res5.layers")

    def load_state_dict(self, state_dict, strict=True, resume=None, **kw):
        if resume is None:
            r = super().load_state_dict(state_dict, strict=strict, **kw)
        else:
            r = self._load_reference_style(dict(state_dict), bool(resume))
        self._prepared = False
        self._graphs, self._pools = {}, {}
        return r

    def _load_reference_style(self, state_dict, resume):
        import warnings
        own = self.state_dict()
        k = "rcnn.cls_score.weight"
        if k in state_dict and own[k].shape[0] == 9 and state_dict[k].shape[0] == 81:
            for wn in ("rcnn.cls_score.weight", "rcnn.cls_score.bias", "rcnn.bbox_pred.weight", "rcnn.bbox_pred.bias",
                       "mask_branch.mask_score.weight", "mask_branch.mask_score.bias"):
                src = state_dict[wn].float()
                mean, std = src.mean().item(), src.std().item()
                src = src.view(*([81, -1] + list(src.shape[1:])))
                blobs = (np.random.randn(*([9] + list(src.shape[1:]))) * std + mean).astype(np.float32)
                for i in range(9):
                    c = self._COCO2CITY_THING[i]
                    if c >= 0:
                        blobs[i] = src[c].cpu().numpy()
                state_dict[wn] = torch.from_numpy(blobs.reshape([-1] + list(src.shape[2:])))
        k = "fcn_head.score.weight"
        if k in own and k in state_dict and own[k].shape[0] == 19 and state_dict[k].shape[0] == 133:
            for wn in ("fcn_head.score.weight", "fcn_head.score.bias"):
                src = state_dict[wn].float()
                mean, std = src.mean().item(), src.std().item()
                blobs = (np.random.randn(*([19] + list(src.shape[1:]))) * std + mean).astype(np.float32)
                for i in range(19):
                    c = self._COCO2CITY_SEG[i]
                    if c >= 0:
                        blobs[i] = src[c].cpu().numpy()
                state_dict[wn] = torch.from_numpy(blobs)
        seen = set()
        with torch.no_grad():
            for name, param in state_dict.items():
                name = self.name_mapping(name, resume)
                seen.add(name)
                if name not in own:
                    warnings.warn('unexpected key "{}" in state_dict'.format(name))
                    continue
                if own[name].shape == param.shape:
                    own[name].copy_(param)
                else:
                    warnings.warn("While copying the parameter named {}, whose dimensions in the models are {} and whose "
                                  "dimensions in the checkpoint are {}, ...".format(name, own[name].size(), param.size()))
        missing = set(own.keys()) - seen
        if missing:
            warnings.warn('missing keys in state_dict: "{}"'.format(missing))
        return None

    def _forward_static(self, x, im_info):
        res2, res3, res4, res5 = self.resnet_backbone(x)
        p2, p3, p4, p5, p6 = self.fpn(res2, res3, res4, res5)
        rpn_cls_prob, rpn_bbox_pred = [], []
        for feat in (p2, p3, p4, p5, p6):
            _, bbox, prob = self.rpn(feat)
            rpn_cls_prob.append(prob)
            rpn_bbox_pred.append(bbox)
        fork = x.is_cuda and self.overlap_heads
        if fork:
            cur = torch.cuda.current_stream(x.device)
# ... 315 lines not shown
```

upsnet_b200/operators.py:

```python
import collections
import ctypes as C
import math

import numpy as np
import torch
import torch.nn as nn
from torch.nn.modules.utils import _pair
from torch.nn.parameter import Parameter

from . import _lib
from ._lib import call, f32c, query_bytes, require_cuda, try_call

_PRECISION = {"conv": _lib.PREC_FP32_SIMT}
DCN_WINDOW = {"on": True, "min_pixels": 4096}
USE_TMA = {"on": True}


def set_precision(name):
    _PRECISION["conv"] = {"fp32": _lib.PREC_FP32_SIMT, "bf16x3": _lib.PREC_BF16X3, "bf16": _lib.PREC_BF16}[name]


def _stream():
    return {_lib.PREC_BF16: "bf16", _lib.PREC_BF16X3: "pair"}.get(_PRECISION["conv"], "f32")

# ... 16 lines not shown
    @property
    def shape(self):
        n, h, w, c2 = self.store.shape
        return torch.Size((n, c2 // 2, h, w))

    @property
    def device(self):
        return self.store.device

    @property
    def is_cuda(self):
        return self.store.is_cuda

    def dim(self):
        return 4

    def size(self, i=None):
        return self.shape if i is None else self.shape[i]

    def float(self):
        c = self.store.shape[-1] // 2
        return (self.store[..., :c].float() + self.store[..., c:].float()).permute(0, 3, 1, 2)

    def record_stream(self, s):
        self.store.record_stream(s)

    def subsample2(self):
        return Pair(self.store[:, ::2, ::2, :].contiguous())


def subsample2(x):
    return x.subsample2() if isinstance(x, Pair) else x[:, :, ::2, ::2].contiguous()


def as_float(x):
    return x.float() if isinstance(x, Pair) else x


STATS = {"launches": 0, "trace": None}


class _Timed:

    def __init__(self, kind, n_kernels, work, device):
        self.kind, self.n, self.work, self.device = kind, n_kernels, work, device
        self.ev = None

    def __enter__(self):
        STATS["launches"] += self.n
        if STATS["trace"] is not None:
            self.ev = (torch.cuda.Event(enable_timing=True), torch.cuda.Event(enable_timing=True))
            self.ev[0].record(torch.cuda.current_stream(self.device))
        return self

    def __exit__(self, *exc):
        if self.ev is not None:
            self.ev[1].record(torch.cuda.current_stream(self.device))
            STATS["trace"].append((self.kind, self.ev[0], self.ev[1], self.work))
        return False


def _conv_out(n, pad, dil, k, stride):
    return (n + 2 * pad - (dil * (k - 1) + 1)) // stride + 1


def _nhwc(x):
    xp = x.permute(0, 2, 3, 1)
    return xp if xp.is_contiguous() else xp.contiguous()


import weakref


def _per_weight(cache, weight, make, device=None, versioned=True):
    hit = cache.get(id(weight))
    if (hit is not None and hit[0]() is weight and (not versioned or hit[1] == weight._version) and
            (device is None or hit[2] is None or hit[2].device == device)):
        return hit[2]
    value = make()
    wid = id(weight)
    cache[wid] = (weakref.ref(weight, lambda _r, _k=wid: cache.pop(_k, None)), weight._version, value)
    return value


_weight_caches = []


def _weight_cache():
    cache = {}
    _weight_caches.append(cache)
    return cache


def forget_packed(tensors):
    ids = [id(t) for t in tensors]
    for cache in _weight_caches:
        for i in ids:
            cache.pop(i, None)


def _packed(cache, weight, pack, nbytes, nbytes_args, unsupported=False):
    def make():
        n = query_bytes(nbytes, *nbytes_args, unsupported=unsupported)
        if n is None:
            return None
        buf = torch.empty(n, dtype=torch.uint8, device=weight.device)
        call(pack, weight.device, f32c(weight.detach()), *weight.shape, buf)
        STATS["launches"] += 1
        return buf
    return _per_weight(cache, weight, make, device=weight.device)


_packed_cache = _weight_cache()


def _packed_weight(weight):
    return _packed(_packed_cache, weight, "igemm_pack_weight", "igemm_packed_weight_bytes", weight.shape)


_dcn_packed_cache = _weight_cache()


def _packed_weight_dcn(weight):
    return _packed(_dcn_packed_cache, weight, "dcn_pack_weight", "dcn_packed_weight_bytes", weight.shape, unsupported=True)


def _dcn_window(x, offset, mask, weight, bias, padding, dilation, relu):
    N, Cin, H, W = x.shape
    if N * H * W < DCN_WINDOW["min_pixels"]:
        return None
    packed = _packed_weight_dcn(weight)
    if packed is None:
        return None
    Cout, _, kh, kw = weight.shape
    ph, pw = padding; dh, dw = dilation
    Ho, Wo = _conv_out(H, ph, dh, kh, 1), _conv_out(W, pw, dw, kw, 1)
    store = torch.empty((N, Ho, Wo, 2 * Cout), device=x.device, dtype=torch.bfloat16)
    work = {"flops": 2.0 * N * Ho * Wo * Cout * Cin * kh * kw * 3, "algo_flops": 2.0 * N * Ho * Wo * Cout * Cin * kh * kw,
            "shape": "N%d %dx%d Cin%d->Cout%d k%d s1 pair->pair (window)" % (N, H, W, Cin, Cout, kh),
            "bytes": float(x.store.numel() * 2 + 4 * weight.numel() + store.numel() * 2 + offset.numel() * 4)}
    with _Timed("dcn", 1, work, x.device):
        rc = try_call("dcn_pair_forward", x.device, x.store, offset, mask, packed, bias, store, N, H, W, Cin, Cout, kh, kw,
                      ph, pw, dh, dw, _lib.EPI_RELU if relu else 0)
    return None if rc == _lib.E_UNSUPPORTED else Pair(store)


_stem_cache = _weight_cache()
_stem_ws = None


def stem_conv(x, weight, bias, padding, relu=True, pair=False):
    global _stem_ws
    require_cuda(x, weight, bias)
    x = f32c(x)
    N, Cin, H, W = x.shape
    Cout, _, kh, kw = weight.shape
    dev = x.device

    packed = _packed(_stem_cache, weight, "stem_pack_weight", "stem_packed_weight_bytes", (Cout, kh))
    nb = query_bytes("stem_workspace_bytes", N, H, W, kh, kw, int(padding))
    if _stem_ws is None:
        _stem_ws = _Workspace()
    ws = _stem_ws.get(dev, nb)
    Ho, Wo = (H + 2 * padding - kh) // 2 + 1, (W + 2 * padding - kw) // 2 + 1
    store = torch.empty((N, Ho, Wo, Cout * (2 if pair else 1)), dtype=torch.bfloat16, device=dev)
    fl = 2.0 * N * Ho * Wo * Cout * Cin * kh * kw
    work = {"flops": fl * (3 if pair else 1), "algo_flops": fl,
            "shape": "N%d %dx%d Cin%d->Cout%d k%d s2 float32->%s (stem, TMA)" % (N, H, W, Cin, Cout, kh, "pair" if pair else "bfloat16"),
            "bytes": float(4 * x.numel() + 2 * store.numel())}
    with _Timed("conv2d", 2, work, dev):
        call("stem_forward", dev, x, packed, None if bias is None else f32c(bias), store, N, Cin, H, W,
             Cout, kh, kw, int(padding), (_lib.EPI_RELU if relu else 0) | (_lib.EPI_STEM_PAIR if pair else 0),
             ws, ws.numel())
    return Pair(store) if pair else store.permute(0, 3, 1, 2)


def _tc_ok(Cin, kh, kw, dg, deform=False):
    return (Cin % 64 == 0 or (Cin <= 8 and not deform)) and dg == 1 and kh * kw <= 49


def _count(n_dev):
    if n_dev is not None:
        assert n_dev.dtype == torch.int32 and n_dev.is_cuda and n_dev.numel() == 1
    return n_dev


def _igemm_tc(kind, x, offset, mask, weight, bias, residual, stride, padding, dilation, relu, prec, out_format,
              out_dtype=None, residual_up2=False, pair_group=0, sigmoid_from=None, n_dev=None):
    sh, sw = stride; ph, pw = padding; dh, dw = dilation
    N, Cin, H, W = x.shape
    Cout, _, kh, kw = weight.shape
    Ho, Wo = _conv_out(H, ph, dh, kh, sh), _conv_out(W, pw, dw, kw, sw)
    nhwc_out = out_format != "nchw"
    x3 = prec == _lib.PREC_BF16X3
    stream = _stream()
    pair_in = isinstance(x, Pair)
    if pair_in:
        assert x3, "Pair activations belong to precision bf16x3"
    elif x3 and stream == "pair" and Cin % 64 == 0:
        x = Pair.from_float(x)
        pair_in = True
    elif x3 and x.dtype != torch.float32:
        x = x.float()
    elif x.dtype not in (torch.float32, torch.bfloat16):
        x = x.float()
    dev = x.device
    pair_out = False
    if out_dtype is None:
        if x3 and stream == "pair" and nhwc_out and Cout % 8 == 0:
            pair_out = True
        else:
            out_dtype = torch.bfloat16 if (stream == "bf16" and prec == _lib.PREC_BF16 and nhwc_out) else torch.float32
    elif out_dtype == "pair":
        pair_out = True
    if pair_in:
        xs, x_dt = x.store, _lib.DTYPE_PAIR
    else:
        xs = f32c(x) if Cin % 64 else _nhwc(x)
        x_dt = _lib.DTYPE_BF16 if xs.dtype == torch.bfloat16 else _lib.DTYPE_F32
    packed = _packed_weight(weight)
    if pair_out:
        assert nhwc_out
        store = torch.empty((N, Ho, Wo, 2 * Cout), device=dev, dtype=torch.bfloat16)
        res = None
        if residual is not None:
            res = (residual if isinstance(residual, Pair) else Pair.from_float(residual)).store
        y_dt = _lib.DTYPE_PAIR
    elif nhwc_out:
        store = torch.empty((N, Ho, Wo, Cout), device=dev, dtype=out_dtype)
        res = None if residual is None else _nhwc(as_float(residual).to(out_dtype))
        y_dt = _lib.DTYPE_BF16 if out_dtype == torch.bfloat16 else _lib.DTYPE_F32
    else:
        store = torch.empty((N, Cout, Ho, Wo), device=dev, dtype=out_dtype)
        res = None if residual is None else as_float(residual).to(out_dtype).contiguous()
        y_dt = _lib.DTYPE_BF16 if out_dtype == torch.bfloat16 else _lib.DTYPE_F32
    xbytes = xs.numel() * xs.element_size()
    work = {"flops": 2.0 * N * Ho * Wo * Cout * Cin * kh * kw * (3 if x3 else 1),
            "algo_flops": 2.0 * N * Ho * Wo * Cout * Cin * kh * kw,
            "shape": "N%d %dx%d Cin%d->Cout%d k%d s%d %s->%s%s" % (N, H, W, Cin, Cout, kh, sh, "pair" if pair_in else str(xs.dtype)[6:],
                                                              "pair" if pair_out else str(out_dtype)[6:],
                                                              " +res" if residual is not None else ""),
            "bytes": float(xbytes + 4 * weight.numel() +
                           store.numel() * store.element_size() * (2 if residual is not None else 1))}
    flags = (_lib.EPI_RELU if relu else 0) | (_lib.EPI_RES_UP2 if residual_up2 else 0) | \
            (0 if USE_TMA["on"] else _lib.EPI_NO_TMA)
    if pair_group:
        assert pair_out and pair_group % 64 == 0 and Cout % pair_group == 0
        flags |= (pair_group // 64) << 8
    if sigmoid_from is not None:
        assert not pair_out and not nhwc_out and residual is None, "sigmoid epilogue: fp32 NCHW head outputs"
        flags |= _lib.EPI_SIGMOID_FROM(sigmoid_from)
    with _Timed(kind, 1, work, dev):
        call("igemm_forward", dev, xs, offset, mask, packed, bias, res,
             store, N, H, W, Cin, Cout, kh, kw, sh, sw, ph, pw, dh, dw,
             _lib.LAYOUT_NHWC if nhwc_out else _lib.LAYOUT_NCHW, x_dt, y_dt, flags,
             prec, _count(n_dev))
    if pair_out:
        if pair_group:
            return Pair(store.view(N, Ho, Wo * (Cout // pair_group), 2 * pair_group))
        return Pair(store)
    return store.permute(0, 3, 1, 2) if nhwc_out else store


def conv2d(x, weight, bias=None, stride=1, padding=0, dilation=1, residual=None, relu=False, precision=None,
           out_format=None, out_dtype=None, residual_up2=False, pair_group=0, sigmoid_from=None, n_dev=None):
    require_cuda(x, weight, bias, residual)
    prec = _PRECISION["conv"] if precision is None else precision
    if prec != _lib.PREC_FP32_SIMT and _tc_ok(weight.shape[1], weight.shape[2], weight.shape[3], 1):
        if residual_up2 and out_format == "nchw":
            residual, residual_up2 = torch.nn.functional.interpolate(as_float(residual), scale_factor=2, mode="nearest"), False
        return _igemm_tc("conv2d", x, None, None, weight, None if bias is None else f32c(bias), residual,
                         _pair(stride), _pair(padding), _pair(dilation), relu, prec, out_format, out_dtype,
                         residual_up2, pair_group, sigmoid_from, n_dev)
    if sigmoid_from is not None:
        y = conv2d(x, weight, bias, stride, padding, dilation, residual, relu, precision, out_format, out_dtype, residual_up2)
        y[:, sigmoid_from:] = torch.sigmoid(y[:, sigmoid_from:])
        return y
    if isinstance(x, Pair):
        x = x.float()
    if isinstance(residual, Pair):
        residual = residual.float()
    if residual_up2:
        residual = torch.nn.functional.interpolate(residual, scale_factor=2, mode="nearest")
    x, weight = f32c(x), f32c(weight)
    bias = None if bias is None else f32c(bias)
    residual = None if residual is None else f32c(residual)
    sh, sw = _pair(stride); ph, pw = _pair(padding); dh, dw = _pair(dilation)
    N, Cin, H, W = x.shape
    Cout, Cin_w, kh, kw = weight.shape
    assert Cin_w == Cin, "groups != 1 is not supported"
    Ho, Wo = _conv_out(H, ph, dh, kh, sh), _conv_out(W, pw, dw, kw, sw)
    y = torch.empty((N, Cout, Ho, Wo), device=x.device, dtype=torch.float32)
    if residual is not None:
        assert residual.shape == y.shape
    prec = _lib.PREC_FP32_SIMT
    work = {"flops": 2.0 * N * Ho * Wo * Cout * Cin * kh * kw, "algo_flops": 2.0 * N * Ho * Wo * Cout * Cin * kh * kw,
            "bytes": 4.0 * (x.numel() + weight.numel() + y.numel() * (2 if residual is not None else 1))}
    with _Timed("conv2d_simt", 1, work, x.device):
        call("conv2d_forward", x.device, x, weight, bias, residual, y, N, Cin, H, W,
             Cout, kh, kw, sh, sw, ph, pw, dh, dw, _lib.EPI_RELU if relu else 0, prec)
    return y


def linear(x, weight, bias=None, relu=False, precision=None, out_dtype=None):
    if isinstance(x, Pair):
        y = conv2d(x, _as_1x1(weight), bias, relu=relu, precision=precision, out_dtype=out_dtype)
        return y if isinstance(y, Pair) else y.reshape(y.shape[0], weight.shape[0])
    N, K = x.shape
    y = conv2d(x.reshape(N, K, 1, 1), _as_1x1(weight), bias, relu=relu, precision=precision, out_dtype=out_dtype)
    return y if isinstance(y, Pair) else y.reshape(N, weight.shape[0])


_view_cache = _weight_cache()


def _as_1x1(weight):
    return _per_weight(_view_cache, weight, lambda: weight.reshape(weight.shape[0], weight.shape[1], 1, 1), versioned=False)


def deform_conv(data, offset, weight, bias=None, stride=1, padding=0, dilation=1, deformable_groups=1,
                mask=None, relu=False, precision=None, out_format=None, out_dtype=None):
    require_cuda(data, offset, weight, bias, mask)
    prec = _PRECISION["conv"] if precision is None else precision
    use_tc = prec != _lib.PREC_FP32_SIMT and _tc_ok(weight.shape[1], weight.shape[2], weight.shape[3], deformable_groups, True)
    offset = f32c(offset)
    bias = None if bias is None else f32c(bias)
    mask = None if mask is None else f32c(mask)
    sh, sw = _pair(stride); ph, pw = _pair(padding); dh, dw = _pair(dilation)
    if use_tc:
        N, Cin, H, W = data.shape
        kh, kw = weight.shape[2], weight.shape[3]
        Ho, Wo = _conv_out(H, ph, dh, kh, sh), _conv_out(W, pw, dw, kw, sw)
        assert tuple(offset.shape) == (N, 2 * kh * kw, Ho, Wo), offset.shape
        if mask is not None:
            assert tuple(mask.shape) == (N, kh * kw, Ho, Wo), mask.shape
        if (DCN_WINDOW["on"] and isinstance(data, Pair) and prec == _lib.PREC_BF16X3 and (sh, sw) == (1, 1) and
                out_format != "nchw" and out_dtype in (None, "pair") and _stream() == "pair"):
            y = _dcn_window(data, offset, mask, weight, bias, (ph, pw), (dh, dw), relu)
            if y is not None:
                return y
        return _igemm_tc("dcn", data, offset, mask, weight, bias, None, (sh, sw), (ph, pw), (dh, dw), relu, prec,
                         out_format, out_dtype)
    data, weight = f32c(as_float(data)), f32c(weight)
    N, Cin, H, W = data.shape
    Cout, Cin_w, kh, kw = weight.shape
    assert Cin_w == Cin, "groups != 1 is not supported (the reference ignores `groups`)"
    Ho, Wo = _conv_out(H, ph, dh, kh, sh), _conv_out(W, pw, dw, kw, sw)
    assert tuple(offset.shape) == (N, 2 * kh * kw * deformable_groups, Ho, Wo), offset.shape
    if mask is not None:
        assert tuple(mask.shape) == (N, kh * kw * deformable_groups, Ho, Wo), mask.shape
    y = torch.empty((N, Cout, Ho, Wo), device=data.device, dtype=torch.float32)
    prec = _lib.PREC_FP32_SIMT
    work = {"flops": 2.0 * N * Ho * Wo * Cout * Cin * kh * kw, "algo_flops": 2.0 * N * Ho * Wo * Cout * Cin * kh * kw,
            "bytes": 4.0 * (data.numel() + offset.numel() + weight.numel() + y.numel() +
                            (mask.numel() if mask is not None else 0))}
    with _Timed("dcn_simt", 1, work, data.device):
        call("dcn_forward", data.device, data, offset, mask, weight, bias, y, N, Cin,
             H, W, Cout, kh, kw, sh, sw, ph, pw, dh, dw, deformable_groups,
             _lib.EPI_RELU if relu else 0, prec)
    return y


def roi_align(features, rois, pooled_height, pooled_width, spatial_scale, sampling_ratio=2, layout="nchw"):
    require_cuda(features, rois)
    features, rois = f32c(features), f32c(rois)
    assert rois.dim() == 2 and rois.shape[1] == 5
    R = rois.shape[0]
    if layout == "nchw":
        B, Cc, H, W = features.shape
        out = torch.empty((R, Cc, pooled_height, pooled_width), device=features.device, dtype=torch.float32)
        lay = _lib.LAYOUT_NCHW
    else:
        B, H, W, Cc = features.shape
        out = torch.empty((R, pooled_height, pooled_width, Cc), device=features.device, dtype=torch.float32)
        lay = _lib.LAYOUT_NHWC
    if R == 0:
        return out
    with _Timed("roi_align", 1, {"bytes": 4.0 * out.numel()}, features.device):
        call("roi_align_forward", features.device, features, B, Cc, H, W, lay, 0, rois, R, pooled_height,
             pooled_width, sampling_ratio, float(spatial_scale), out)
    return out


def max_pool2d(x, kernel_size, stride, padding):
    require_cuda(x)
    N, Cc, H, W = x.shape
    Ho = (H + 2 * padding - kernel_size) // stride + 1
    Wo = (W + 2 * padding - kernel_size) // stride + 1
    if isinstance(x, Pair):
        store = torch.empty((N, Ho, Wo, 2 * Cc), device=x.device, dtype=torch.bfloat16)
        with _Timed("maxpool", 1, {"bytes": float((x.store.numel() + store.numel()) * 2)}, x.device):
            call("maxpool2d_nhwc", x.device, x.store, store, N, H, W, Cc, kernel_size, stride, padding, _lib.DTYPE_PAIR)
        return Pair(store)
    if x.dtype not in (torch.float32, torch.bfloat16):
        x = x.float()
    xs = _nhwc(x)
    store = torch.empty((N, Ho, Wo, Cc), device=x.device, dtype=x.dtype)
    with _Timed("maxpool", 1, {"bytes": float((xs.numel() + store.numel()) * x.element_size())}, x.device):
        call("maxpool2d_nhwc", x.device, xs, store, N, H, W, Cc, kernel_size, stride, padding,
             1 if x.dtype == torch.bfloat16 else 0)
    return store.permute(0, 3, 1, 2)


def upsample_bilinear(x, factor):
    require_cuda(x)
    x = f32c(x)
    N, Cc, H, W = x.shape
    y = torch.empty((N, Cc, H * factor, W * factor), dtype=torch.float32, device=x.device)
    with _Timed("upsample", 1, {"bytes": 4.0 * (x.numel() + y.numel())}, x.device):
        call("upsample_bilinear_nchw", x.device, x, y, N * Cc, H, W, int(factor))
    return y


def fcn_score_fuse(s2, s3, s4, s5):
    require_cuda(s2, s3, s4, s5)
    s2, s3, s4, s5 = f32c(s2), f32c(s3), f32c(s4), f32c(s5)
    N, Cc, H, W = s2.shape
    assert s3.shape == (N, Cc, H // 2, W // 2) and s4.shape == (N, Cc, H // 4, W // 4) and s5.shape == (N, Cc, H // 8, W // 8)
    out = torch.empty_like(s2)
    with _Timed("upsample", 1, {"bytes": 4.0 * (2 * s2.numel() + s3.numel() + s4.numel() + s5.numel())}, s2.device):
        call("fcn_score_fuse", s2.device, s2, s3, s4, s5, out, N * Cc, H, W)
    return out


def _gn_store(x, like=None):
    if like is not None:
        if like.dtype == "pair":
            x = x if isinstance(x, Pair) else Pair.from_float(x)
        else:
            x = as_float(x).to(like.dtype)
    if isinstance(x, Pair):
        return x.store, _lib.DTYPE_PAIR
    if x.dtype not in (torch.float32, torch.bfloat16):
        x = x.float()
    return _nhwc(x), (_lib.DTYPE_BF16 if x.dtype == torch.bfloat16 else _lib.DTYPE_F32)


def _gn_wrap(store, dt):
    return Pair(store) if dt == _lib.DTYPE_PAIR else store.permute(0, 3, 1, 2)


def group_norm(x, weight, bias, groups=32, eps=1e-5, relu=False, residual=None, residual_up2=False, shift=None,
               return_stats=False):
    require_cuda(x, weight, bias, shift)
    if (residual is not None) != bool(residual_up2):
        raise _lib.UpsnetError("group_norm: a residual is read with nearest 2x up-sampling only (residual_up2=True)")
    N, C, H, W = x.shape
    xs, dt = _gn_store(x)
    res = None if residual is None else _gn_store(residual, like=xs if dt != _lib.DTYPE_PAIR else x)[0]
    y = torch.empty_like(xs)
    stats = torch.empty((N, groups, 2), dtype=torch.float32, device=xs.device)
    ws = torch.empty(query_bytes("group_norm_workspace_bytes", N, C, H, W, groups), dtype=torch.uint8, device=xs.device)
    nbytes = xs.numel() * xs.element_size()
    work = {"bytes": float(3 * nbytes + (0 if res is None else res.numel() * res.element_size())),
            "shape": "N%d %dx%d C%d G%d %s%s%s" % (N, H, W, C, groups, {0: "float32", 1: "bfloat16", 2: "pair"}[dt],
                                                  " +res" if res is not None else "", " +shift" if shift is not None else "")}
    flags = (_lib.EPI_RELU if relu else 0) | (_lib.EPI_RES_UP2 if res is not None else 0)
    with _Timed("group_norm", 3, work, xs.device):
        call("group_norm_forward", xs.device, xs, f32c(weight), f32c(bias), None if shift is None else f32c(shift), res,
             y, stats, N, C, H, W, groups, float(eps), dt, flags, ws, ws.numel())
    out = _gn_wrap(y, dt)
    return (out, stats) if return_stats else out


def group_norm_rows(x, weight, bias, groups=32, eps=1e-5, relu=False, n_dev=None):
    require_cuda(x, weight, bias)
    flat = not isinstance(x, Pair) and x.dim() == 2
    xs, dt = _gn_store(x.reshape(x.shape[0], x.shape[1], 1, 1) if flat else x)
    R, h, w, _ = xs.shape
    C = weight.shape[0]
    y = torch.empty_like(xs)
    work = {"bytes": float(2 * xs.numel() * xs.element_size()),
            "shape": "R%d %dx%d C%d G%d rows" % (R, h, w, C, groups)}
    with _Timed("group_norm", 1, work, xs.device):
        call("group_norm_rows", xs.device, xs, f32c(weight), f32c(bias), y, R, C, h * w, groups, float(eps), dt,
             _lib.EPI_RELU if relu else 0, _count(n_dev))
    return y.reshape(R, C) if flat else _gn_wrap(y, dt)


def fpn_roi_align(feats, rois, pooled_height, pooled_width, spatial_scales, sampling_ratio=2, layout="nchw",
                  return_levels=False, n_dev=None):
    assert len(feats) == 4 and len(spatial_scales) == 4
    require_cuda(rois, *feats)
    rois = f32c(rois)
    R = rois.shape[0]
    if isinstance(feats[0], Pair):
        assert all(isinstance(f, Pair) for f in feats) and layout in ("auto", "nhwc", "flat_pair") and not return_levels
        B, Cc = feats[0].shape[0], feats[0].shape[1]
        flat = layout == "flat_pair"
        if flat:
            out = torch.empty((R, 1, 1, 2 * pooled_height * pooled_width * Cc), device=rois.device, dtype=torch.bfloat16)
        else:
            out = torch.empty((R, pooled_height, pooled_width, 2 * Cc), device=rois.device, dtype=torch.bfloat16)
        if R > 0:
            fp = (C.c_void_p * 4)(*[f.store.data_ptr() for f in feats])
            hs = (C.c_int * 4)(*[f.shape[2] for f in feats]); ws = (C.c_int * 4)(*[f.shape[3] for f in feats])
            sc = (C.c_float * 4)(*[float(s_) for s_ in spatial_scales])
            with _Timed("roi_align_fpn", 1, {"bytes": 2.0 * out.numel()}, rois.device):
                call("roi_align_fpn_forward", rois.device, fp, hs, ws, sc, B, Cc,
                     _lib.LAYOUT_FLAT_PAIR if flat else _lib.LAYOUT_NHWC, _lib.DTYPE_PAIR, rois, R, pooled_height,
                     pooled_width, sampling_ratio, out, None, _count(n_dev))
        return Pair(out)
    if layout == "auto":
        cl = all(f.dim() == 4 and f.permute(0, 2, 3, 1).is_contiguous() and not f.is_contiguous() for f in feats)
        if cl:
            out = fpn_roi_align([f.permute(0, 2, 3, 1) for f in feats], rois, pooled_height, pooled_width,
                                spatial_scales, sampling_ratio, "nhwc", return_levels)
            return (out[0].permute(0, 3, 1, 2), out[1]) if return_levels else out.permute(0, 3, 1, 2)
        layout = "nchw"
    bf16 = layout == "nhwc" and all(f.dtype == torch.bfloat16 for f in feats)
    feats = [f.contiguous() for f in feats] if bf16 else [f32c(f) for f in feats]
    odt = torch.bfloat16 if bf16 else torch.float32
    if layout == "nchw":
        B, Cc = feats[0].shape[0], feats[0].shape[1]
        Hs = [f.shape[2] for f in feats]; Ws = [f.shape[3] for f in feats]
        out = torch.empty((R, Cc, pooled_height, pooled_width), device=rois.device, dtype=torch.float32)
        lay = _lib.LAYOUT_NCHW
    else:
        B, Cc = feats[0].shape[0], feats[0].shape[3]
        Hs = [f.shape[1] for f in feats]; Ws = [f.shape[2] for f in feats]
        out = torch.empty((R, pooled_height, pooled_width, Cc), device=rois.device, dtype=odt)
        lay = _lib.LAYOUT_NHWC
    assert n_dev is None, "fpn_roi_align: the roi count bound is implemented for pair features"
    levels = torch.empty((R,), device=rois.device, dtype=torch.int32) if return_levels else None
    fp = (C.c_void_p * 4)(*[f.data_ptr() for f in feats])
    hs = (C.c_int * 4)(*Hs); ws = (C.c_int * 4)(*Ws)
    sc = (C.c_float * 4)(*[float(s) for s in spatial_scales])
    with _Timed("roi_align_fpn", 1, {"bytes": 4.0 * out.numel()}, rois.device):
        call("roi_align_fpn_forward", rois.device, fp, hs, ws, sc, B, Cc, lay, 1 if bf16 else 0, rois, R, pooled_height,
             pooled_width, sampling_ratio, out, levels, None)
    return (out, levels) if return_levels else out


import threading


class _WsSlot(threading.local):
    i = 0

    def __getitem__(self, k):
        assert k == "i"
        return self.i

    def __setitem__(self, k, v):
        assert k == "i"
        self.i = int(v)


WS_SLOT = _WsSlot()


class _Workspace:

    def __init__(self):
        self.buf = {}
        self.retired = []

    def get(self, device, nbytes):
        key = (device, WS_SLOT["i"])
        b = self.buf.get(key)
        if b is None or b.numel() < nbytes:
            if b is not None:
                self.retired.append(b)
                nbytes = max(int(nbytes), int(b.numel() * 1.5))
            b = torch.empty(max(int(nbytes), 1), dtype=torch.uint8, device=device)
            self.buf[key] = b
        return b


_nms_ws = _Workspace()
_nms_ws_side = _Workspace()
_pan_ws = _Workspace()


def nms_segmented(boxes_sorted, seg_offsets, max_seg_len, thresh, side=False):
    require_cuda(boxes_sorted, seg_offsets)
    boxes_sorted = f32c(boxes_sorted)
    assert seg_offsets.dtype == torch.int32
    S = seg_offsets.numel() - 1
    dev = boxes_sorted.device
    nbytes = query_bytes("nms_workspace_bytes", S, max_seg_len)
    ws = (_nms_ws_side if side else _nms_ws).get(dev, nbytes)
    keep = torch.empty((S, max_seg_len), dtype=torch.int32, device=dev)
    cnt = torch.empty((S,), dtype=torch.int32, device=dev)
    with _Timed("nms", 2, {"bytes": 20.0 * boxes_sorted.shape[0]}, dev):
        call("nms_segmented", dev, boxes_sorted, seg_offsets, S, max_seg_len, float(thresh), keep, cnt, ws, ws.numel())
    return keep, cnt


def im_info_device(im_info, dev):
    if torch.is_tensor(im_info) and im_info.device == torch.device(dev) and im_info.dtype == torch.float32:
        assert im_info.numel() == 3, "im_info: one (h, w, scale) row"
        return im_info.reshape(3)
    t = im_info.detach().cpu() if torch.is_tensor(im_info) else torch.from_numpy(np.asarray(im_info, dtype=np.float32))
    t = t.to(torch.float32).reshape(-1)[:3].contiguous()
    if torch.device(dev).type != "cuda":
        return t.to(dev)
    return t.pin_memory().to(dev, non_blocking=True)


def rpn_decode(bbox_preds, top_idx, shapes, strides, base_anchors, A, im_info):
    L = len(bbox_preds)
    dev = bbox_preds[0].device
    require_cuda(*bbox_preds, *top_idx, base_anchors)
    assert base_anchors.dtype == torch.float64 and base_anchors.is_contiguous()
    bbox_preds = [f32c(b) for b in bbox_preds]
# ... 767 lines not shown
```

Measured before the change: 128.7.

## Fuse 1x1 head conv into TMA implicit-GEMM epilogue for RPN and mask heads

Adds a head variant of the TMA/wgmma implicit-GEMM kernel in which each CTA processes all N-tiles of a head group consecutively. It runs a second small wgmma of the ReLU'd tile against the packed 1x1 head weights and accumulates across tiles in registers or parked shared memory. The epilogue applies bias and sigmoid and writes fp32 output directly, including the 2x2 pixel shuffle for the mask head, so the intermediate feature map is never written to or read from global memory. The cost is a fixed BN of 128, extra shared-memory stages for the head weights, and fewer parallel work items, which is why a heuristic gate on SM count falls back to the old two-conv path.

New measurement: 128.9 (median of 6 runs). About the same (+0.2%).

```diff
diff --git a/include/upsnet_b200.h b/include/upsnet_b200.h
--- a/include/upsnet_b200.h
+++ b/include/upsnet_b200.h
@@ -69,6 +69,10 @@
                          int N, int H, int W, int Cin, int Cout, int kh, int kw, int stride_h,
                          int stride_w, int pad_h, int pad_w, int dil_h, int dil_w, int out_layout,
                          int x_dtype, int y_dtype, int epi_flags, int precision, const int *n_dev, void *stream);
+int upsnet_igemm_head_forward(const void *x_nhwc, const void *packed, const float *bias, const void *head_packed,
+                              const float *head_bias, float *head_y, int N, int H, int W, int Cin, int Cout, int kh, int kw,
+                              int pad_h, int pad_w, int head_group, int head_cout, int sigmoid_from, int shuffle,
+                              int epi_flags, int precision, const int *n_dev, void *stream);
 int upsnet_tma_set_tile_n(int bn);
 
 int upsnet_dcn_packed_weight_bytes(int Cout, int Cin, int kh, int kw, size_t *bytes);
diff --git a/upsnet_b200/csrc/capi.cu b/upsnet_b200/csrc/capi.cu
--- a/upsnet_b200/csrc/capi.cu
+++ b/upsnet_b200/csrc/capi.cu
@@ -127,3 +127,34 @@
   if (p.y_pair && !p.out_nhwc) return UPSNET_E_BADARG;
   return ups::launch_igemm_tc(p, packed, (cudaStream_t)stream);
 }
+
+extern "C" int upsnet_igemm_head_forward(const void* x_nhwc, const void* packed, const float* bias, const void* head_packed,
+                                         const float* head_bias, float* head_y, int N, int H, int W, int Cin, int Cout,
+                                         int kh, int kw, int pad_h, int pad_w, int head_group, int head_cout,
+                                         int sigmoid_from, int shuffle, int epi_flags, int precision, const int* n_dev,
+                                         void* stream) {
+  if (!x_nhwc || !packed || !head_packed || !head_y) return UPSNET_E_BADARG;
+  if (N <= 0 || Cin <= 0 || H <= 0 || W <= 0 || Cout <= 0 || kh <= 0 || kw <= 0 || pad_h < 0 || pad_w < 0 ||
+      head_group <= 0 || Cout % head_group || head_cout <= 0 || sigmoid_from < -1 || sigmoid_from >= head_cout)
+    return UPSNET_E_BADARG;
+  if (precision != UPSNET_PREC_BF16X3 && precision != UPSNET_PREC_BF16) return UPSNET_E_BADARG;
+  if ((size_t)H * W >= (1ull << 31)) return UPSNET_E_UNSUPPORTED;
+  ups::TcParams p{};
+  p.x = x_nhwc; p.bias = bias; p.n_dev = n_dev;
+  p.N = N; p.H = H; p.W = W; p.Cin = Cin; p.Cout = Cout; p.kh = kh; p.kw = kw;
+  p.sh = 1; p.sw = 1; p.ph = pad_h; p.pw = pad_w; p.dh = 1; p.dw = 1;
+  p.Ho = ups::conv_out_size(H, pad_h, 1, kh, 1);
+  p.Wo = ups::conv_out_size(W, pad_w, 1, kw, 1);
+  if (p.Ho <= 0 || p.Wo <= 0) return UPSNET_E_BADARG;
+  if (shuffle && Cout / head_group != 4) return UPSNET_E_BADARG;
+  p.relu = (epi_flags & UPSNET_EPI_RELU) ? 1 : 0;
+  p.sig_from = -1;
+  p.x3 = precision == UPSNET_PREC_BF16X3;
+  p.x_pair = p.y_pair = p.x3;
+  p.x_bf16 = p.y_bf16 = !p.x3;
+  p.out_nhwc = 1;
+  p.y = head_y;
+  p.pair_group = p.x3 ? head_group : 0;
+  const ups::TmaHead head{head_packed, head_bias, head_y, head_group, head_cout, sigmoid_from, shuffle ? 1 : 0};
+  return ups::launch_igemm_tma(p, packed, (cudaStream_t)stream, &head);
+}
diff --git a/upsnet_b200/csrc/igemm_tma.cu b/upsnet_b200/csrc/igemm_tma.cu
--- a/upsnet_b200/csrc/igemm_tma.cu
+++ b/upsnet_b200/csrc/igemm_tma.cu
@@ -14,6 +14,7 @@
 constexpr int TM_MAX_STAGES = 8;
 constexpr int TM_SLAB_BYTES = 128 * 128;
 constexpr int TM_MMA_BF16 = 0, TM_MMA_WIDE = 1;
+constexpr int TM_HEAD_C = 32;
 
 struct TmaGeom {
   const float* bias;
@@ -35,7 +36,15 @@
   int res_inplace;
   int opairs;
   int wide;
+  int tpg;
+  int hG, hCout, hsig, hshuf;
+  const float* hbias;
+  float* hy;
 };
+
+__device__ __forceinline__ long long tile_next(long long t, int tpg) {
+  return (t + 1) % tpg ? t + 1 : t + 1 + (long long)(gridDim.x - 1) * tpg;
+}
 
 __device__ __forceinline__ int pair_chan(int n, int G) { return (n / G) * 2 * G + (n % G); }
 
@@ -92,10 +101,9 @@
   return s;
 }
 
-template <int N, int MMA>
-__global__ void __launch_bounds__(TM_THREADS, 1)
-igemm_tma_kernel(const __grid_constant__ CUtensorMap tm_x, const __grid_constant__ CUtensorMap tm_w,
-                 const __grid_constant__ CUtensorMap tm_y, const __grid_constant__ CUtensorMap tm_r, const TmaGeom g) {
+template <int N, int MMA, int HN>
+__device__ __forceinline__ void igemm_tma_body(const CUtensorMap& tm_x, const CUtensorMap& tm_w, const CUtensorMap& tm_y,
+                                               const CUtensorMap& tm_r, const TmaGeom& g) {
   extern __shared__ __align__(1024) uint8_t smem_dyn[];
   const uint32_t raw = smem_u32(smem_dyn);
   const uint32_t base = (raw + 1023u) & ~1023u;
@@ -112,6 +120,7 @@
   const long long m_tiles = (long long)g.tiles_w * g.tiles_h * tiles_n;
   const long long num_tiles = m_tiles * g.n_tiles;
   const uint32_t box_bytes = (uint32_t)(g.bw * g.bh * g.bn) * 128u;
+  const int tpg = HN > 0 ? g.tpg : 1;
 
   if (tid == 0) {
     for (int s = 0; s < g.stages; ++s) {
@@ -136,7 +145,7 @@
       uint32_t s = 0, ph = 0;
       uint32_t a_dst = base + L.stages;
       const uint32_t tx_bytes = (g.x3 ? 2u * box_bytes : box_bytes) + L.b_bytes;
-      for (long long tile = blockIdx.x; tile < num_tiles; tile += gridDim.x) {
+      for (long long tile = (long long)blockIdx.x * tpg; tile < num_tiles; tile = tile_next(tile, tpg)) {
         const int nt = (int)(tile % g.n_tiles);
         const long long mt = tile / g.n_tiles;
         const int w0 = (int)(mt % g.tiles_w) * g.bw;
@@ -169,6 +178,18 @@
           a_dst += L.stage_bytes;
           if (++s == (uint32_t)g.stages) { s = 0; ph ^= 1u; a_dst = base + L.stages; }
         }
+        if constexpr (HN > 0) {
+          const uint32_t bf = bar_full + 8 * s;
+          mbar_wait(bar_empty + 8 * s, ph ^ 1u);
+          mbar_arrive_expect_tx(bf, (uint32_t)(g.BN / 64) * HN * 128u);
+          for (int sl = 0; sl < g.BN / 64; ++sl) {
+            const int kc = n0 % g.hG + 64 * sl;
+            tma_load_2d(a_dst + (uint32_t)sl * HN * 128u, &tm_r, bf, kc, 0);
+            if constexpr (MMA == TM_MMA_WIDE) tma_load_2d(a_dst + (uint32_t)sl * HN * 128u + (HN / 2) * 128u, &tm_r, bf, kc, 32);
+          }
+          a_dst += L.stage_bytes;
+          if (++s == (uint32_t)g.stages) { s = 0; ph ^= 1u; a_dst = base + L.stages; }
+        }
       }
     }
     __syncwarp();
@@ -176,7 +197,7 @@
     if (lane == 0 && g.has_res) {
       uint32_t ti_local = 0;
       const int slabs = g.BN / 64;
-      for (long long tile = blockIdx.x; tile < num_tiles; tile += gridDim.x, ++ti_local) {
+      for (long long tile = (long long)blockIdx.x * tpg; tile < num_tiles; tile = tile_next(tile, tpg), ++ti_local) {
         const int nt = (int)(tile % g.n_tiles);
         const long long mt = tile / g.n_tiles;
         const int w0 = (int)(mt % g.tiles_w) * g.bw;
@@ -276,8 +297,81 @@
       const int r = wg * 64 + 16 * (warp & 3) + (lane >> 2) + 8 * h, rr = res_row(r);
       fr_row[h] = (uint32_t)r * 128u; fr_res[h] = (uint32_t)rr * 128u; fr_rx[h] = (uint32_t)(rr & 7);
     }
+    constexpr int HC = MMA == TM_MMA_WIDE ? HN / 2 : HN;
+    float dh[HN > 0 ? HN / 2 : 1];
+    uint32_t hst = 0, hs = 0;
+    auto head_mma = [&](uint32_t a_hi, uint32_t a_lo, uint32_t bw, bool first) {
+      if constexpr (HN > 0) {
+        const uint32_t a = wg_desc_lo(a_hi + a_row0), al = wg_desc_lo(a_lo + a_row0), b = wg_desc_lo(bw);
+        wgmma_fence();
+#pragma unroll
+        for (uint32_t k = 0; k < 4; ++k) {
+          const uint32_t acc = (first && k == 0) ? 0u : 1u;
+          if constexpr (MMA == TM_MMA_WIDE) {
+            Wgmma<HN>::mma(dh, wg_desc(a + 2 * k, dhi), wg_desc(b + 2 * k, dhi), acc);
+            Wgmma<HN / 2>::mma(*reinterpret_cast<float(*)[HN / 4]>(&dh[0]), wg_desc(al + 2 * k, dhi), wg_desc(b + 2 * k, dhi), 1u);
+          } else {
+            Wgmma<HN>::mma(dh, wg_desc(a + 2 * k, dhi), wg_desc(b + 2 * k, dhi), acc);
+          }
+        }
+        wgmma_commit();
+        wgmma_wait<0>();
+        wgmma_fence_acc(dh);
+      }
+    };
+    auto head_park = [&](bool store) {
+      if constexpr (HN > 0 && MMA == TM_MMA_WIDE) {
+#pragma unroll
+        for (int j = 0; j < HN / 8; ++j) {
+          const uint32_t a = base + L.out + (uint32_t)(j * 256 + tid) * 16u;
+          if (store) {
+            asm volatile("st.shared.v4.f32 [%0], {%1, %2, %3, %4};" ::"r"(a), "f"(dh[4 * j]), "f"(dh[4 * j + 1]), "f"(dh[4 * j + 2]),
+                         "f"(dh[4 * j + 3]) : "memory");
+          } else {
+            asm volatile("ld.shared.v4.f32 {%0, %1, %2, %3}, [%4];"
+                         : "=f"(dh[4 * j]), "=f"(dh[4 * j + 1]), "=f"(dh[4 * j + 2]), "=f"(dh[4 * j + 3]) : "r"(a) : "memory");
+          }
+        }
+      }
+    };
+    auto head_end = [&](int nt, int w0, int h0, int i0) {
+      if constexpr (HN > 0) {
+        __syncwarp();
+        if (lane == 0) mbar_arrive(bar_empty + 8 * hs);
+        if ((nt + 1) % g.tpg) return;
+        if constexpr (MMA == TM_MMA_WIDE) {
+#pragma unroll
+          for (int i = 0; i < HN / 4; ++i) dh[i] += dh[HN / 4 + i];
+        }
+        float* hbuf = reinterpret_cast<float*>(sm + L.out);
+        named_bar(5, 256);
+        acc_stage_sw<HN, HC>(dh, hbuf, wg * 64);
+        named_bar(5, 256);
+        const int hrow = (warp & 3) * 32 + lane;
+        const int wq = hrow % g.bw, hq = (hrow / g.bw) % g.bh, nq = hrow / (g.bw * g.bh);
+        const int wo = w0 + wq, ho = h0 + hq, ni = i0 + nq;
+        if (nq >= g.bn || wo >= g.Wo || ho >= g.Ho || ni >= g.N) return;
+        const int grp = nt / g.tpg, K = g.hCout;
+        const size_t HoWo = (size_t)g.Ho * g.Wo;
+        const size_t cs = g.hshuf ? 4 * HoWo : HoWo;
+        const size_t y0 = g.hshuf ? (size_t)ni * K * cs + (size_t)(2 * ho + (grp >> 1)) * 2 * g.Wo + 2 * wo + (grp & 1)
+                                  : (size_t)ni * K * cs + (size_t)ho * g.Wo + wo;
+        const int cb = (warp >> 2) * (HC / 2);
+        uint32_t v[16];
+        acc_ld16_sw(smem_u32(hbuf + (size_t)hrow * HC), hrow, cb, v);
+#pragma unroll
+        for (int e = 0; e < HC / 2; ++e) {
+          const int co = cb + e;
+          if (co >= K) break;
+          float o = __uint_as_float(v[e]);
+          if (g.hbias) o += __ldg(g.hbias + co);
+          if (g.hsig >= 0 && co >= g.hsig) o = 1.f / (1.f + expf(-o));
+          g.hy[y0 + (size_t)co * cs] = o;
+        }
+      }
+    };
     uint32_t ti_local = 0, oc = 0;
-    for (long long tile = blockIdx.x; tile < num_tiles; tile += gridDim.x, ++ti_local) {
+    for (long long tile = (long long)blockIdx.x * tpg; tile < num_tiles; tile = tile_next(tile, tpg), ++ti_local) {
       const int nt = (int)(tile % g.n_tiles);
       const long long mt = tile / g.n_tiles;
       const int w0 = (int)(mt % g.tiles_w) * g.bw;
@@ -286,6 +380,13 @@
       const int n0 = nt * g.BN;
       const uint32_t buf = ti_local & 1u, use = ti_local >> 1;
       mainloop();
+      if constexpr (HN > 0) {
+        mbar_wait(bar_full + 8 * s, ph);
+        hst = base + L.stages + s * L.stage_bytes;
+        hs = s;
+        if (++s == (uint32_t)g.stages) { s = 0; ph ^= 1u; }
+      }
+      const bool hfirst = HN > 0 && nt % g.tpg == 0;
       if (g.has_res) mbar_wait(bar_rfull + 8 * buf, use & 1u);
       if (g.direct) {
         const int wq = row % g.bw, hq = (row / g.bw) % g.bh, nq = row / (g.bw * g.bh);
@@ -318,6 +419,7 @@
         const bool lead = warp == 0 && lane == 0;
         const uint32_t cq4 = (uint32_t)(lane & 3) * 4u;
         const uint32_t fx = (uint32_t)(lane >> 2);
+        head_park(false);
 #pragma unroll
         for (int sl = 0; sl < SW / 64; ++sl, ++oc) {
           uint32_t ob;
@@ -360,7 +462,9 @@
           }
           fence_proxy_async();
           named_bar(1, 256);
-          if (lead) {
+          if constexpr (HN > 0) {
+            head_mma(ob, ob + TM_SLAB_BYTES, hst + (uint32_t)sl * HN * 128u, hfirst && sl == 0);
+          } else if (lead) {
             const int c = pair_chan(n0 + sl * 64, g.pg);
             tma_store_4d(&tm_y, ob, c, w0, h0, i0);
             tma_store_4d(&tm_y, ob + TM_SLAB_BYTES, c + g.pg, w0, h0, i0);
@@ -373,6 +477,11 @@
           bulk_wait_read0();
           mbar_arrive(bar_rempty + 8 * buf);
         }
+        if (HN > 0 && (nt + 1) % g.tpg) {
+          named_bar(1, 256);
+          head_park(true);
+        }
+        head_end(nt, w0, h0, i0);
       } else {
         for (int ui = 0; ui < upw; ++ui) {
           const int u = half * upw + ui;
@@ -418,7 +527,7 @@
           if ((u & 1) == 1 || g.BN == 64) {
             fence_proxy_async();
             named_bar(bar_id, bar_cnt);
-            if (leader) {
+            if (HN == 0 && leader) {
               tma_store_4d(&tm_y, out_slab, n0 + slab * 64, w0, h0, i0);
               bulk_commit();
             }
@@ -426,10 +535,30 @@
         }
         __syncwarp();
         if (lane == 0 && g.has_res) mbar_arrive(bar_rempty + 8 * buf);
+        if constexpr (HN > 0) {
+          named_bar(4, 256);
+#pragma unroll
+          for (int sl = 0; sl < N / 64; ++sl)
+            head_mma(base + L.out + (uint32_t)sl * TM_SLAB_BYTES, 0u, hst + (uint32_t)sl * HN * 128u, hfirst && sl == 0);
+          head_end(nt, w0, h0, i0);
+        }
       }
     }
     if (leader || (g.x3 && warp == 0 && lane == 0)) bulk_wait0();
   }
+}
+
+template <int N, int MMA>
+__global__ void __launch_bounds__(TM_THREADS, 1)
+igemm_tma_kernel(const __grid_constant__ CUtensorMap tm_x, const __grid_constant__ CUtensorMap tm_w,
+                 const __grid_constant__ CUtensorMap tm_y, const __grid_constant__ CUtensorMap tm_r, const TmaGeom g) {
+  igemm_tma_body<N, MMA, 0>(tm_x, tm_w, tm_y, tm_r, g);
+}
+template <int N, int MMA>
+__global__ void __launch_bounds__(TM_THREADS, 1)
+igemm_tma_head_kernel(const __grid_constant__ CUtensorMap tm_x, const __grid_constant__ CUtensorMap tm_w,
+                      const __grid_constant__ CUtensorMap tm_y, const __grid_constant__ CUtensorMap tm_r, const TmaGeom g) {
+  igemm_tma_body<N, MMA, MMA == TM_MMA_WIDE ? 2 * TM_HEAD_C : TM_HEAD_C>(tm_x, tm_w, tm_y, tm_r, g);
 }
 
 static bool encode_bf16(EncodeTiledFn enc, CUtensorMap* tm, const void* ptr, int rank, const cuuint64_t* dims,
@@ -466,18 +595,27 @@
   *bw_o = bbw; *bh_o = bbh; *bn_o = bbn;
 }
 
-template <int N, int MMA>
+template <int N, int MMA, bool HEAD = false>
 static int tma_launch_n(dim3 grid, size_t smem, cudaStream_t stream, const CUtensorMap& tm_x, const CUtensorMap& tm_w,
                         const CUtensorMap& tm_y, const CUtensorMap& tm_r, const TmaGeom& g) {
+  auto kernel = [] {
+    if constexpr (HEAD) return igemm_tma_head_kernel<N, MMA>;
+    else return igemm_tma_kernel<N, MMA>;
+  }();
   static ups::PerDeviceOnce configured;
   if (configured.need())
-    UPS_CUDA(cudaFuncSetAttribute(igemm_tma_kernel<N, MMA>, cudaFuncAttributeMaxDynamicSharedMemorySize, 227 * 1024));
-  igemm_tma_kernel<N, MMA><<<grid, TM_THREADS, smem, stream>>>(tm_x, tm_w, tm_y, tm_r, g);
+    UPS_CUDA(cudaFuncSetAttribute(kernel, cudaFuncAttributeMaxDynamicSharedMemorySize, 227 * 1024));
+  kernel<<<grid, TM_THREADS, smem, stream>>>(tm_x, tm_w, tm_y, tm_r, g);
   UPS_CHECK_LAUNCH();
   return 0;
 }
 static int tma_launch(int BN, dim3 grid, size_t smem, cudaStream_t stream, const CUtensorMap& tm_x, const CUtensorMap& tm_w,
                       const CUtensorMap& tm_y, const CUtensorMap& tm_r, const TmaGeom& g) {
+  if (g.hy) {
+    if (BN != 128) return UPSNET_E_UNSUPPORTED;
+    if (g.wide) return tma_launch_n<256, TM_MMA_WIDE, true>(grid, smem, stream, tm_x, tm_w, tm_y, tm_r, g);
+    return tma_launch_n<128, TM_MMA_BF16, true>(grid, smem, stream, tm_x, tm_w, tm_y, tm_r, g);
+  }
   if (g.wide) {
     if (BN == 32) return tma_launch_n<64, TM_MMA_WIDE>(grid, smem, stream, tm_x, tm_w, tm_y, tm_r, g);
     if (BN == 64) return tma_launch_n<128, TM_MMA_WIDE>(grid, smem, stream, tm_x, tm_w, tm_y, tm_r, g);
@@ -507,8 +645,11 @@
 
 static int g_tma_force_bn = 0;
 
-int launch_igemm_tma(const TcParams& p, const void* packed, cudaStream_t stream) {
+int launch_igemm_tma(const TcParams& p, const void* packed, cudaStream_t stream, const TmaHead* head) {
   if (p.no_tma || p.offset) return UPSNET_E_UNSUPPORTED;
+  if (head && (p.residual || p.sh != 1 || p.sw != 1 || head->G % 128 || p.Cout % head->G || head->Cout <= 0 || head->Cout > TM_HEAD_C ||
+               !head->y || !head->packed || (((uintptr_t)head->packed) & 15) || (head->bias && (((uintptr_t)head->bias) & 15))))
+    return UPSNET_E_UNSUPPORTED;
   const bool pair = p.x_pair != 0;
   if (pair != (p.x3 != 0) || (!pair && !p.x_bf16)) return UPSNET_E_UNSUPPORTED;
   if (p.y_pair && (!pair || !p.out_nhwc || (p.Cout % 64) != 0)) return UPSNET_E_UNSUPPORTED;
@@ -544,7 +685,9 @@
   g.x3 = pair ? 1 : 0; g.x_lo = p.Cin; g.w_lo = Cout_pad; g.pg = pg;
   g.res_inplace = (pair && g.has_res && !g.res_up2) ? 1 : 0;
   g.opairs = 2;
-  if (g_tma_force_bn && Cout_pad % g_tma_force_bn == 0) {
+  if (head) {
+    BN = 128;
+  } else if (g_tma_force_bn && Cout_pad % g_tma_force_bn == 0) {
     BN = g_tma_force_bn;
   } else {
     while (BN > 64 && m_tiles * (Cout_pad / BN) < 88) BN /= 2;
@@ -552,13 +695,19 @@
   g.direct = direct ? 1 : 0; g.y_bf16 = p.y_bf16; g.out_nhwc = p.out_nhwc; g.y = p.y;
   TmaSmem L;
   bool ok = tma_fit(BN, g.has_res != 0, direct, pair, g.res_up2 != 0, g.res_inplace != 0, &g.stages, &g.opairs, &L);
-  while (BN > 64 && (!ok || (pair && g.stages < 3))) {
+  while (!head && BN > 64 && (!ok || (pair && g.stages < 3))) {
     BN /= 2;
     ok = tma_fit(BN, g.has_res != 0, direct, pair, g.res_up2 != 0, g.res_inplace != 0, &g.stages, &g.opairs, &L);
   }
-  if (!ok) return UPSNET_E_UNSUPPORTED;
+  if (!ok || (head && pair && g.stages < 3)) return UPSNET_E_UNSUPPORTED;
   g.BN = BN;
   g.n_tiles = Cout_pad / BN;
+  g.tpg = 1;
+  if (head) {
+    g.tpg = head->G / BN;
+    g.hG = head->G; g.hCout = head->Cout; g.hsig = head->sig_from; g.hshuf = head->shuffle;
+    g.hbias = head->bias; g.hy = head->y;
+  }
 
   const int Kp = g.KHW * p.Cin;
   CUtensorMap tm_x, tm_w, tm_y, tm_r;
@@ -577,6 +726,11 @@
     if (direct) {
       tm_y = tm_x;
       tm_r = tm_x;
+    } else if (head) {
+      tm_y = tm_x;
+      const cuuint64_t dh[2] = {(cuuint64_t)head->G, 64};
+      const cuuint32_t boxh[2] = {64, (cuuint32_t)TM_HEAD_C};
+      if (!encode_bf16(enc, &tm_r, head->packed, 2, dh, boxh)) return UPSNET_E_UNSUPPORTED;
     } else {
     if (!encode_bf16(enc, &tm_y, p.y, 4, dy, box)) return UPSNET_E_UNSUPPORTED;
     if (g.res_up2) {
@@ -591,7 +745,8 @@
   const long long num_tiles = m_tiles * g.n_tiles;
   if (num_tiles <= 0) return 0;
   g.wide = pair ? 1 : 0;
-  dim3 grid((unsigned)(num_tiles < sms ? num_tiles : sms));
+  const long long items = num_tiles / g.tpg;
+  dim3 grid((unsigned)(items < sms ? items : sms));
   return tma_launch(BN, grid, L.total + 1024, stream, tm_x, tm_w, tm_y, tm_r, g);
 }
 
@@ -699,7 +854,7 @@
   g.relu = (epi_flags & UPSNET_EPI_RELU) ? 1 : 0;
   g.sig_from = -1;
   g.stem = 1; g.y = y; g.y_bf16 = 1; g.out_nhwc = 1;
-  g.x3 = pair ? 1 : 0; g.w_lo = Cout; g.pg = Cout; g.opairs = 2; g.x_lo = 0;
+  g.x3 = pair ? 1 : 0; g.w_lo = Cout; g.pg = Cout; g.opairs = 2; g.x_lo = 0; g.tpg = 1;
   tma_pick_box(N, Ho, Wo, 1, 1, 1, 1, false, &g.bw, &g.bh, &g.bn);
   g.tiles_w = (Wo + g.bw - 1) / g.bw;
   g.tiles_h = (Ho + g.bh - 1) / g.bh;
diff --git a/upsnet_b200/csrc/tc_params.cuh b/upsnet_b200/csrc/tc_params.cuh
--- a/upsnet_b200/csrc/tc_params.cuh
+++ b/upsnet_b200/csrc/tc_params.cuh
@@ -50,6 +50,10 @@
 int tc_pack_weight(const float* w, int Cout, int Cin, int kh, int kw, void* packed, cudaStream_t stream);
 bool tc_supported(int Cin, int kh, int kw, int dg);
 int launch_igemm_tc(TcParams p, const void* packed, cudaStream_t stream);
-int launch_igemm_tma(const TcParams& p, const void* packed, cudaStream_t stream);
+struct TmaHead {
+  const void* packed; const float* bias; float* y;
+  int G, Cout, sig_from, shuffle;
+};
+int launch_igemm_tma(const TcParams& p, const void* packed, cudaStream_t stream, const TmaHead* head = nullptr);
 
 }
diff --git a/upsnet_b200/model.py b/upsnet_b200/model.py
--- a/upsnet_b200/model.py
+++ b/upsnet_b200/model.py
@@ -350,9 +350,12 @@
 
     def forward(self, x):
         c = self.conv_proposal[0]
-        t = ops.conv2d(x, c.weight, c.bias, padding=1, relu=True)
         A = self.num_anchors
-        both = ops.conv2d(t, self._f[0], self._f[1], out_format="nchw", sigmoid_from=5 * A).float()
+        if ops.conv2d_head_ok(x, self._f[0].shape[0]):
+            both = ops.conv2d_head(x, c.weight, c.bias, self._f[0], self._f[1], padding=1, relu=True, sigmoid_from=5 * A)
+        else:
+            t = ops.conv2d(x, c.weight, c.bias, padding=1, relu=True)
+            both = ops.conv2d(t, self._f[0], self._f[1], out_format="nchw", sigmoid_from=5 * A).float()
         return both[:, :A], both[:, A:5 * A], both[:, 5 * A:]
 
     def forward_train(self, x, prec):
@@ -467,6 +470,9 @@
             if self.gn:
                 x = ops.group_norm_rows(x, c[1].weight, c[1].bias, c[1].num_groups, c[1].eps, relu=True, n_dev=n_dev)
         w1, b1, cout = self._f
+        if ops.conv2d_head_ok(x, self.mask_score.weight.shape[0], groups=4):
+            return ops.conv2d_head(x, w1, b1, self.mask_score.weight, self.mask_score.bias, relu=True, group=cout,
+                                   shuffle=True, **bound)
         if isinstance(x, ops.Pair):
             yv = ops.conv2d(x, w1, b1, relu=True, pair_group=cout, **bound)
             n, _, h, w4 = yv.shape
diff --git a/upsnet_b200/operators.py b/upsnet_b200/operators.py
--- a/upsnet_b200/operators.py
+++ b/upsnet_b200/operators.py
@@ -342,6 +342,61 @@
     return y
 
 
+HEAD_MAX_COUT = 32
+_SMS = {}
+
+
+def _num_sms(dev):
+    if dev not in _SMS:
+        _SMS[dev] = torch.cuda.get_device_properties(dev).multi_processor_count
+    return _SMS[dev]
+
+
+def conv2d_head_ok(x, head_cout, groups=1, precision=None):
+    if not _head_stream_ok(x, head_cout, precision):
+        return False
+    N, _, H, W = x.shape
+    return -(-N * H * W // 128) * groups >= _num_sms(x.device)
+
+
+def _head_stream_ok(x, head_cout, precision=None):
+    prec = _PRECISION["conv"] if precision is None else precision
+    if not USE_TMA["on"] or head_cout > HEAD_MAX_COUT:
+        return False
+    if isinstance(x, Pair):
+        return prec == _lib.PREC_BF16X3
+    return prec == _lib.PREC_BF16 and x.is_cuda and x.dtype == torch.bfloat16
+
+
+def conv2d_head(x, weight, bias, head_weight, head_bias, padding=0, relu=False, group=None, sigmoid_from=None,
+                shuffle=False, n_dev=None):
+    require_cuda(weight, bias, head_weight, head_bias)
+    prec = _PRECISION["conv"]
+    assert _head_stream_ok(x, head_weight.shape[0]), "conv2d_head: pair or bf16 stream on the TMA kernel, head <= %d channels" \
+        % HEAD_MAX_COUT
+    N, Cin, H, W = x.shape
+    Cout, _, kh, kw = weight.shape
+    K, G = head_weight.shape[0], group or Cout
+    assert head_weight.shape[1:] == (G, 1, 1) and Cout % G == 0 and (not shuffle or Cout == 4 * G)
+    ph, pw = _pair(padding)
+    Ho, Wo = _conv_out(H, ph, 1, kh, 1), _conv_out(W, pw, 1, kw, 1)
+    dev = weight.device
+    xs = x.store if isinstance(x, Pair) else _nhwc(x)
+    y = torch.empty((N, K, 2 * Ho, 2 * Wo) if shuffle else (N, K, Ho, Wo), device=dev, dtype=torch.float32)
+    fl = 2.0 * N * Ho * Wo * Cout * (Cin * kh * kw + K)
+    work = {"flops": fl * (3 if prec == _lib.PREC_BF16X3 else 1), "algo_flops": fl,
+            "shape": "N%d %dx%d Cin%d->Cout%d k%d s1 %s->head %dx%d->%d%s" % (
+                N, H, W, Cin, Cout, kh, "pair" if isinstance(x, Pair) else "bfloat16", Cout // G, G, K,
+                " shuffle" if shuffle else ""),
+            "bytes": float(xs.numel() * xs.element_size() + 4 * weight.numel() + 4 * y.numel())}
+    with _Timed("conv2d", 1, work, dev):
+        call("igemm_head_forward", dev, xs, _packed_weight(weight), None if bias is None else f32c(bias),
+             _packed_weight(head_weight), None if head_bias is None else f32c(head_bias), y, N, H, W, Cin, Cout, kh, kw,
+             ph, pw, G, K, -1 if sigmoid_from is None else int(sigmoid_from), 1 if shuffle else 0,
+             _lib.EPI_RELU if relu else 0, prec, _count(n_dev))
+    return y
+
+
 def linear(x, weight, bias=None, relu=False, precision=None, out_dtype=None):
     if isinstance(x, Pair):
         y = conv2d(x, _as_1x1(weight), bias, relu=relu, precision=precision, out_dtype=out_dtype)
```
